# ChenKaiXuSan/Skiing_Analysis_PyTorch

Measured on AMD Instinct MI355X. Metric: 3D-pose frames/sec, 8-view 518px clips, higher is better.
Workload: dtype f16

## Files before the change

include/skimi.h:

```cpp
#ifndef SKIMI_H
#define SKIMI_H

#include <stddef.h>
#include <stdint.h>

#ifdef __cplusplus
extern "C" {
#endif

#define SKIMI_OK 0
#define SKIMI_ERR_ARG (-1)
#define SKIMI_ERR_HIP (-2)
#define SKIMI_ERR_STATE (-3)
#define SKIMI_ERR_WORKSPACE (-4)

#define SKIMI_F32 0
#define SKIMI_BF16 1
#define SKIMI_BF16X3_REC 2
#define SKIMI_FP8MX 3
#define SKIMI_F16 4

#define SKIMI_PREC_BF16 0
#define SKIMI_PREC_BF16X3 1
#define SKIMI_PREC_FP8 2
#define SKIMI_PREC_F16 3

#define SKIMI_ACT_NONE 0
#define SKIMI_ACT_RELU 1
#define SKIMI_ACT_GELU 2
#define SKIMI_ACT_SILU 3
#define SKIMI_ACT_SIGMOID 4

const char* skimi_last_error(void);
int skimi_version(void);
int skimi_sizeof_gemm_desc(void);
int skimi_device_count(void);

int skimi_profile_start(int32_t kind, int64_t min_size);
int skimi_profile_stop(double* total_ms, int64_t* launches, double* flops, double* bytes);

typedef struct skimi_gemm_desc {
    int32_t M, N, K;
    const void* A;
    const void* W;
    int32_t a_dtype, w_dtype;
    int64_t lda, ldw;
    int32_t prec;
    int32_t a_mode;
    int32_t cN, cH, cW, cC, KH, KW, stride, pad, dil, OH, OW;
    const float* bias;
    const float* gamma;
    const void* resid;
    int32_t resid_dtype;
    int64_t ldr;
    int32_t resid_rows_per_batch;
    int64_t resid_batch_stride;
    int64_t resid_row_off;
    int32_t act;
    const void* resid2;
    int64_t ldr2;
    int32_t post_act;
    int32_t out_rows_per_batch;
    int64_t out_batch_stride;
    int64_t out_row_off;
    void* out;
    void* out2;
    int32_t out_dtype;
    int64_t ldo, ldo2;
    int32_t store_mode, ps_s, ps_C;
    void* splitk_scratch;
    uint64_t splitk_scratch_bytes;
    int32_t force_splitk;
    int32_t splitk_scratch_zeroed;
    const void* W_split;
    void* x3_scratch;
    uint64_t x3_scratch_bytes;
    void* out_records;
} skimi_gemm_desc;

int skimi_split_planes(const float* x, int64_t ld, int64_t rows, int32_t C, void* hi, void* lo, void* stream);

int skimi_split_records(const float* x, int64_t ld, int64_t rows, int32_t C, void* records, void* stream);

int skimi_dpt_fold_pack(const float* w_T, const float* b_T, const float* w_rn, int32_t C_in, int32_t C_mid, int32_t C_out,
                        int32_t s, void* w_records, float* beta, void* stream);

int skimi_gemm(const skimi_gemm_desc* d, void* stream);

#define SKIMI_GEMM_PATH_GENERIC 1
#define SKIMI_GEMM_PATH_SPLITK_ORDERED 2
#define SKIMI_GEMM_PATH_SPLITK_ATOMIC 3
#define SKIMI_GEMM_PATH_X3DMA_WIDE 4
#define SKIMI_GEMM_PATH_X3DMA_NARROW 5
#define SKIMI_GEMM_PATH_GEMM256 6
#define SKIMI_GEMM_PATH_CONV_WIN 7
int32_t skimi_gemm_last_path(void);

int skimi_quant_mx(const void* x, int32_t dtype, int64_t ldx, int64_t rows, int32_t K, void* payload, void* scales,
                   void* stream);
int skimi_layernorm_mx(const float* x, int64_t ldx, int64_t rows, int32_t C, const float* gamma, const float* beta,
                       float eps, void* payload, void* scales, void* stream);
int skimi_gemm_fp8(const void* A, const void* A_scales, const void* W, const void* W_scales, int32_t M, int32_t N,
                   int32_t K, const float* bias, int32_t act, const float* gamma, const float* resid, int64_t ldr,
                   void* out, int32_t out_dtype, int64_t ldo, void* out_scales, void* stream);

int skimi_conv3x3_n32_pack(const float* w, void* packed, int32_t C, void* stream);
int skimi_conv3x3_n32(const void* in_hi, const void* in_lo, const void* packed_w, const float* bias, float* out,
                      int32_t F, int32_t H, int32_t W, int32_t C, int32_t relu, void* stream);

int skimi_resample_u8(const uint8_t* in, uint8_t* out, int64_t outer, int32_t n_in, int32_t n_out, int64_t inner,
                      const int32_t* kk, const int32_t* bounds, int32_t ksize, void* stream);
int skimi_u8_hwc_to_f32_chw(const uint8_t* in, int32_t H, int32_t W, float* out, int32_t OH, int32_t OW, int32_t y_off,
                            int32_t x_off, float fill, void* stream);

int skimi_layernorm(const float* x, const float* x2, int64_t ldx, int64_t rows, int32_t C,
                    const float* gamma, const float* beta, float eps,
                    void* out, int32_t out_dtype, int64_t ldo, void* stream);

int skimi_qknorm_rope(void* qkv, int32_t dtype, int64_t tokens, int32_t heads,
                      const float* qn_w, const float* qn_b, const float* kn_w, const float* kn_b,
                      float eps, const int32_t* pos, const float* rope_cos, const float* rope_sin,
                      int32_t rope_npos, void* stream);

int skimi_attention(const void* qkv, void* out, int32_t dtype, int32_t batch, int32_t seq,
                    int32_t heads, int32_t head_dim, void* stream);
int skimi_attention_out(const void* qkv, void* out, int32_t dtype, int32_t out_dtype, int32_t batch, int32_t seq,
                        int32_t heads, int32_t head_dim, void* stream);

int skimi_qknorm_rope_scaled(void* qkv, int32_t dtype, int64_t tokens, int32_t heads,
                             const float* qn_w, const float* qn_b, const float* kn_w, const float* kn_b,
                             float eps, const int32_t* pos, const float* rope_cos, const float* rope_sin,
                             int32_t rope_npos, float q_scale, int32_t* q_scaled, void* stream);
int skimi_attention_ex(const void* qkv, void* out, int32_t dtype, int32_t out_dtype, int32_t batch, int32_t seq,
                       int32_t heads, int32_t head_dim, int32_t q_prescaled, void* x3_scratch,
                       uint64_t x3_scratch_bytes, int32_t* out_records, void* stream);
uint64_t skimi_attention_x3_scratch_bytes(int64_t tokens, int64_t row_elems);

typedef struct skimi_vp3d skimi_vp3d;

skimi_vp3d* skimi_vp3d_create(int32_t joints_in, int32_t in_features, int32_t joints_out,
                              const int32_t* filter_widths, int32_t n_widths,
                              int32_t channels, int32_t causal);
skimi_vp3d* skimi_vp3d_create_ex(int32_t joints_in, int32_t in_features, int32_t joints_out,
                                 const int32_t* filter_widths, int32_t n_widths,
                                 int32_t channels, int32_t causal, int32_t dense);
void skimi_vp3d_destroy(skimi_vp3d*);
int skimi_vp3d_set_weight(skimi_vp3d*, const char* key, const float* host_data, int64_t n);
int skimi_vp3d_finalize(skimi_vp3d*, int32_t prec);
int32_t skimi_vp3d_receptive_field(const skimi_vp3d*);
size_t skimi_vp3d_workspace_bytes(const skimi_vp3d*, int32_t batch, int32_t frames_in);
int skimi_vp3d_forward(skimi_vp3d*, const float* x, float* out, int32_t batch, int32_t frames_in,
                       void* workspace, size_t workspace_bytes, void* stream);

typedef struct skimi_vggt skimi_vggt;

typedef struct skimi_vggt_config {
    int32_t patch_size, embed_dim, depth, num_heads, num_register_tokens;
    int32_t use_dino;
    int32_t dino_depth, dino_heads, dino_img_size;
    int32_t cam_trunk_depth, cam_heads, cam_iters;
// ... 96 lines not shown
```

skiing_analysis_pytorch_amd/_lib.py:

```python
from __future__ import annotations

import ctypes as C
from pathlib import Path

LIB_PATH = Path(__file__).resolve().parent / "lib" / "libskimi.so"

F32, BF16 = 0, 1
F16 = 4
BF16X3_REC = 2
FP8MX = 3
PREC_BF16, PREC_BF16X3, PREC_FP8 = 0, 1, 2
PREC_F16 = 3
ACT_NONE, ACT_RELU, ACT_GELU, ACT_SILU, ACT_SIGMOID = 0, 1, 2, 3, 4
GEMM_PATH_GENERIC, GEMM_PATH_SPLITK_ORDERED, GEMM_PATH_SPLITK_ATOMIC = 1, 2, 3
GEMM_PATH_X3DMA_WIDE, GEMM_PATH_X3DMA_NARROW, GEMM_PATH_GEMM256, GEMM_PATH_CONV_WIN = 4, 5, 6, 7


class SkimiError(RuntimeError):
    pass


class GemmDesc(C.Structure):

    _fields_ = [
        ("M", C.c_int32), ("N", C.c_int32), ("K", C.c_int32),
        ("A", C.c_void_p), ("W", C.c_void_p),
        ("a_dtype", C.c_int32), ("w_dtype", C.c_int32),
        ("lda", C.c_int64), ("ldw", C.c_int64),
        ("prec", C.c_int32),
        ("a_mode", C.c_int32),
        ("cN", C.c_int32), ("cH", C.c_int32), ("cW", C.c_int32), ("cC", C.c_int32),
        ("KH", C.c_int32), ("KW", C.c_int32), ("stride", C.c_int32), ("pad", C.c_int32),
        ("dil", C.c_int32), ("OH", C.c_int32), ("OW", C.c_int32),
        ("bias", C.c_void_p), ("gamma", C.c_void_p), ("resid", C.c_void_p),
        ("resid_dtype", C.c_int32),
        ("ldr", C.c_int64),
        ("resid_rows_per_batch", C.c_int32),
        ("resid_batch_stride", C.c_int64),
        ("resid_row_off", C.c_int64),
        ("act", C.c_int32),
        ("resid2", C.c_void_p), ("ldr2", C.c_int64), ("post_act", C.c_int32),
        ("out_rows_per_batch", C.c_int32), ("out_batch_stride", C.c_int64), ("out_row_off", C.c_int64),
        ("out", C.c_void_p), ("out2", C.c_void_p),
        ("out_dtype", C.c_int32),
        ("ldo", C.c_int64), ("ldo2", C.c_int64),
        ("store_mode", C.c_int32), ("ps_s", C.c_int32), ("ps_C", C.c_int32),
        ("splitk_scratch", C.c_void_p),
        ("splitk_scratch_bytes", C.c_uint64),
        ("force_splitk", C.c_int32), ("splitk_scratch_zeroed", C.c_int32),
        ("W_split", C.c_void_p), ("x3_scratch", C.c_void_p), ("x3_scratch_bytes", C.c_uint64),
        ("out_records", C.c_void_p),
    ]


_vp = C.c_void_p
_SIGNATURES = {
    "skimi_last_error": (C.c_char_p, []),
    "skimi_version": (C.c_int, []),
    "skimi_sizeof_gemm_desc": (C.c_int, []),
    "skimi_device_count": (C.c_int, []),
    "skimi_profile_start": (C.c_int, [C.c_int32, C.c_int64]),
    "skimi_profile_stop": (C.c_int, [C.POINTER(C.c_double), C.POINTER(C.c_int64), C.POINTER(C.c_double),
                                    C.POINTER(C.c_double)]),
    "skimi_gemm": (C.c_int, [C.POINTER(GemmDesc), _vp]),
    "skimi_gemm_last_path": (C.c_int32, []),
    "skimi_dpt_fold_pack": (C.c_int, [_vp, _vp, _vp, C.c_int32, C.c_int32, C.c_int32, C.c_int32, _vp, _vp, _vp]),
    "skimi_quant_mx": (C.c_int, [_vp, C.c_int32, C.c_int64, C.c_int64, C.c_int32, _vp, _vp, _vp]),
    "skimi_layernorm_mx": (C.c_int, [_vp, C.c_int64, C.c_int64, C.c_int32, _vp, _vp, C.c_float, _vp, _vp, _vp]),
    "skimi_gemm_fp8": (C.c_int, [_vp, _vp, _vp, _vp, C.c_int32, C.c_int32, C.c_int32, _vp, C.c_int32, _vp, _vp, C.c_int64,
                                 _vp, C.c_int32, C.c_int64, _vp, _vp]),
    "skimi_split_planes": (C.c_int, [_vp, C.c_int64, C.c_int64, C.c_int32, _vp, _vp, _vp]),
    "skimi_split_records": (C.c_int, [_vp, C.c_int64, C.c_int64, C.c_int32, _vp, _vp]),
    "skimi_resample_u8": (C.c_int, [_vp, _vp, C.c_int64, C.c_int32, C.c_int32, C.c_int64, _vp, _vp, C.c_int32, _vp]),
    "skimi_u8_hwc_to_f32_chw": (C.c_int, [_vp, C.c_int32, C.c_int32, _vp, C.c_int32, C.c_int32, C.c_int32, C.c_int32,
                                          C.c_float, _vp]),
    "skimi_conv3x3_n32_pack": (C.c_int, [_vp, _vp, C.c_int32, _vp]),
    "skimi_conv3x3_n32": (C.c_int, [_vp, _vp, _vp, _vp, _vp, C.c_int32, C.c_int32, C.c_int32, C.c_int32, C.c_int32, _vp]),
    "skimi_layernorm": (C.c_int, [_vp, _vp, C.c_int64, C.c_int64, C.c_int32, _vp, _vp, C.c_float, _vp,
                                  C.c_int32, C.c_int64, _vp]),
    "skimi_qknorm_rope": (C.c_int, [_vp, C.c_int32, C.c_int64, C.c_int32, _vp, _vp, _vp, _vp, C.c_float,
                                    _vp, _vp, _vp, C.c_int32, _vp]),
    "skimi_attention": (C.c_int, [_vp, _vp, C.c_int32, C.c_int32, C.c_int32, C.c_int32, C.c_int32, _vp]),
    "skimi_attention_out": (C.c_int, [_vp, _vp, C.c_int32, C.c_int32, C.c_int32, C.c_int32, C.c_int32, C.c_int32, _vp]),
    "skimi_qknorm_rope_scaled": (C.c_int, [_vp, C.c_int32, C.c_int64, C.c_int32, _vp, _vp, _vp, _vp, C.c_float,
                                           _vp, _vp, _vp, C.c_int32, C.c_float, C.POINTER(C.c_int32), _vp]),
    "skimi_attention_ex": (C.c_int, [_vp, _vp, C.c_int32, C.c_int32, C.c_int32, C.c_int32, C.c_int32, C.c_int32, C.c_int32,
                                     _vp, C.c_uint64, C.POINTER(C.c_int32), _vp]),
    "skimi_attention_x3_scratch_bytes": (C.c_uint64, [C.c_int64, C.c_int64]),
    "skimi_vp3d_create": (_vp, [C.c_int32, C.c_int32, C.c_int32, C.POINTER(C.c_int32), C.c_int32,
                                C.c_int32, C.c_int32]),
    "skimi_vp3d_create_ex": (_vp, [C.c_int32, C.c_int32, C.c_int32, C.POINTER(C.c_int32), C.c_int32,
                                   C.c_int32, C.c_int32, C.c_int32]),
    "skimi_vp3d_destroy": (None, [_vp]),
    "skimi_vp3d_set_weight": (C.c_int, [_vp, C.c_char_p, _vp, C.c_int64]),
    "skimi_vp3d_finalize": (C.c_int, [_vp, C.c_int32]),
    "skimi_vp3d_receptive_field": (C.c_int32, [_vp]),
    "skimi_vp3d_workspace_bytes": (C.c_size_t, [_vp, C.c_int32, C.c_int32]),
    "skimi_vp3d_forward": (C.c_int, [_vp, _vp, _vp, C.c_int32, C.c_int32, _vp, C.c_size_t, _vp]),
    "skimi_pose_to_cameras": (C.c_int, [_vp, C.c_int64, C.c_int32, C.c_int32, _vp, _vp, _vp]),
    "skimi_unproject_depth": (C.c_int, [_vp, _vp, _vp, _vp, C.c_int32, C.c_int32, C.c_int32, _vp]),
    "skimi_triangulate_dlt": (C.c_int, [_vp, _vp, _vp, _vp, _vp, C.c_int64, C.c_int32, C.c_int32, _vp]),
    "skimi_triangulate_triage": (C.c_int, [_vp, _vp, _vp, _vp, _vp, C.c_double, C.c_double, C.c_int64, C.c_int32, C.c_int32,
                                           _vp, _vp, _vp, _vp, _vp, _vp, _vp, _vp]),
    "skimi_triangulate_robust": (C.c_int, [_vp, _vp, _vp, _vp, _vp, C.c_double, C.c_double, C.c_int32, C.c_int32, C.c_int32,
                                           C.c_int64, C.c_int32, C.c_int32, _vp, _vp, _vp, _vp, _vp, _vp, _vp, _vp, _vp]),
    "skimi_person_workspace_bytes": (C.c_size_t, [C.c_int64, C.c_int32, C.c_int32]),
    "skimi_person_origin": (C.c_int, [_vp, _vp, C.c_int64, C.c_int32, C.c_int32, C.c_int32, C.c_int32, _vp, _vp, _vp]),
    "skimi_recenter_cameras": (C.c_int, [_vp, _vp, C.c_int64, C.c_int32, _vp, _vp, _vp, _vp]),
    "skimi_icp_workspace_bytes": (C.c_size_t, [C.c_int64, C.c_int64]),
    "skimi_estimate_normals": (C.c_int, [_vp, C.c_int64, C.c_double, _vp, _vp, _vp, C.c_size_t, _vp]),
    "skimi_icp_correspondences": (C.c_int, [_vp, C.c_int64, _vp, C.c_int64, C.POINTER(C.c_double), C.c_double, _vp, _vp,
                                            C.c_size_t, _vp]),
    "skimi_icp_point_to_plane": (C.c_int, [_vp, C.c_int64, _vp, C.c_int64, C.c_double, C.c_double, C.c_int32, C.c_double,
                                           C.c_double, C.POINTER(C.c_double), C.POINTER(C.c_double), C.POINTER(C.c_double),
                                           C.POINTER(C.c_double), C.POINTER(C.c_int32), _vp, C.c_size_t, _vp]),
    "skimi_ba_workspace_bytes": (C.c_size_t, [C.c_int64, C.c_int32, C.c_int32, C.c_int32]),
    "skimi_bundle_adjust": (C.c_int, [_vp, _vp, _vp, _vp, _vp, _vp, C.c_int64, C.c_int32, C.c_int32, C.POINTER(C.c_int32),
                                      C.c_int32, C.c_int32, C.c_double, C.c_double, C.c_double, C.c_double, C.c_double,
                                      C.c_double, C.c_int32, _vp, _vp, _vp, _vp, _vp, C.c_size_t, _vp]),
    "skimi_resect_workspace_bytes": (C.c_size_t, [C.c_int64, C.c_int32, C.c_int64]),
    "skimi_resect_cameras": (C.c_int, [_vp, _vp, _vp, _vp, _vp, _vp, C.c_int64, C.c_int32, C.c_int64, C.c_int32, C.c_double,
                                       C.c_double, C.c_int32, _vp, _vp, _vp, _vp, _vp, _vp, _vp, _vp, _vp, _vp, _vp, C.c_size_t,
                                       _vp]),
    "skimi_relative_pose": (C.c_int, [_vp, _vp, C.c_int64, C.c_int32, _vp, _vp, _vp]),
    "skimi_vggt_create": (_vp, [_vp]),
    "skimi_vggt_destroy": (None, [_vp]),
    "skimi_vggt_set_weight": (C.c_int, [_vp, C.c_char_p, _vp, C.c_int64, C.c_int32]),
    "skimi_vggt_finalize": (C.c_int, [_vp]),
    "skimi_vggt_set_pos_embed": (C.c_int, [_vp, C.c_int32, C.c_int32, _vp, C.c_int32]),
    "skimi_vggt_rope_positions": (C.c_int, [_vp, C.c_int32, C.c_int32, C.c_int32, _vp]),
    "skimi_vggt_workspace_bytes": (C.c_size_t, [_vp, C.c_int32, C.c_int32, C.c_int32, C.c_int32, C.c_int32]),
    "skimi_vggt_forward": (C.c_int, [_vp, _vp, _vp, C.c_int32, C.c_int32, C.c_int32, C.c_int32, C.c_int32, _vp,
                                     _vp, C.c_size_t, _vp]),
}
# ... 51 lines not shown
```

skiing_analysis_pytorch_amd/csrc/gemm.hip:

```cpp
#include "common.h"
#include "gemm_epilogue.h"
#include <algorithm>
#include <stdlib.h>

namespace skimi {

#define SKIMI_ENV_FLAG(NAME) ([]() { static const bool v = getenv(NAME) && atoi(getenv(NAME)); return v; }())

template <typename T> struct Stage;
template <> struct Stage<float> { float4 a, b; };
template <> struct Stage<unsigned short> { bf16x8 v; };

__device__ __forceinline__ void stage_load(Stage<float>& s, const float* p) {
    s.a = *reinterpret_cast<const float4*>(p);
    s.b = *reinterpret_cast<const float4*>(p + 4);
}
__device__ __forceinline__ void stage_load(Stage<unsigned short>& s, const unsigned short* p) {
    s.v = *reinterpret_cast<const bf16x8*>(p);
}
__device__ __forceinline__ void stage_mask(Stage<float>& s, bool ok) {
    s.a.x = ok ? s.a.x : 0.f; s.a.y = ok ? s.a.y : 0.f; s.a.z = ok ? s.a.z : 0.f; s.a.w = ok ? s.a.w : 0.f;
    s.b.x = ok ? s.b.x : 0.f; s.b.y = ok ? s.b.y : 0.f; s.b.z = ok ? s.b.z : 0.f; s.b.w = ok ? s.b.w : 0.f;
}
__device__ __forceinline__ void stage_mask(Stage<unsigned short>& s, bool ok) {
// ... 317 lines not shown
        if (p.splitk_ordered) {
            for (int sk = 1; sk < p.splitk; ++sk) {
                float* q = p.partial + (long)sk * total + idx;
                v += *q;
                *q = 0.f;
            }
        }
        store_one(p, rm, n, v);
    }
}

template <int BM, int BN, int BK, int NSPLIT, typename TA, typename TW, bool F16 = false>
static int launch_cfg(const GemmArgs& a, hipStream_t st) {
    constexpr int DEPTH = (BM == 64 && BN == 64) ? 4 : 1;
    constexpr int NPL = (NSPLIT == 3) ? 2 : 1;
    constexpr size_t lds = 2ull * NPL * (BM + BN) * BK * 2;
    auto kfn = gemm_kernel<BM, BN, BK, NSPLIT, TA, TW, DEPTH, F16>;
    SKIMI_LDS_OPT_IN(kfn, lds, "gemm");
    dim3 grid(a.ntm * a.ntn, a.splitk);
    hipLaunchKernelGGL(kfn, grid, dim3(256), lds, st, a);
    SKIMI_LAUNCH_CHECK();
    return SKIMI_OK;
}

static thread_local int tl_gemm_path = 0;
void set_gemm_path(int family, int tile, int mfma, int epi, int splitk) {
    tl_gemm_path = family | (tile << 4) | (mfma << 8) | (epi << 12) | (splitk << 16);
}
int gemm_last_path() { return tl_gemm_path; }

int gemm_dispatch(const skimi_gemm_desc* d, hipStream_t st, void* scratch, size_t scratch_bytes,
                  int force_splitk) {
    tl_gemm_path = 0;
    SKIMI_CHECK_ARG(d != nullptr, "skimi_gemm: null descriptor");
    SKIMI_CHECK_ARG(d->M > 0 && d->N > 0 && d->K > 0, "skimi_gemm: empty shape M=%d N=%d K=%d", d->M, d->N, d->K);
    SKIMI_CHECK_ARG(d->K % 8 == 0, "skimi_gemm: K=%d must be a multiple of 8", d->K);
    SKIMI_CHECK_ARG(d->A && d->W && (d->out || d->out_records), "skimi_gemm: null buffer");
    const bool fold = d->a_mode == 3 || d->store_mode == 2;
    if (fold) {
        SKIMI_CHECK_ARG(d->a_mode == 3 && d->store_mode == 2, "skimi_gemm: a_mode 3 and store_mode 2 come together");
        SKIMI_CHECK_ARG(d->cC > 0 && d->cC % 32 == 0 && d->K == 4 * d->cC && (long)d->cN * d->cH * d->cW == d->M &&
                            d->ps_s >= 2 && d->N == d->ps_C && d->N % 32 == 0 && d->lda >= d->cC,
                        "skimi_gemm: bad phase-folded geometry (K = 4 cC, M = cN cH cW, N = ps_C, ps_s >= 2)");
        SKIMI_CHECK_ARG(gemm_x3dma_eligible(d),
                        "skimi_gemm: the phase-folded ConvTranspose + 3x3 conv runs on the 256-column LDS-DMA bf16x3 kernel only "
                        "(W_split, the 9-class bias table, fp32 out / records, ReLU or no activation, ps_C > 128, cW >= 2, a "
                        "chip's worth of tiles)");
    }
    if (d->out_records) {
        SKIMI_CHECK_ARG(d->N % 32 == 0 && (d->store_mode == 0 || fold) && d->out_rows_per_batch == 0 && d->out_row_off == 0 &&
                            d->out2 == nullptr && ((uintptr_t)d->out_records & 127) == 0,
                        "skimi_gemm: out_records needs N %% 32 == 0, plain output rows, no out2, 128-byte alignment");
        SKIMI_CHECK_ARG(d->out || d->out_dtype == SKIMI_F32, "skimi_gemm: records-only output is written from fp32 results");
        SKIMI_CHECK_ARG(d->prec == SKIMI_PREC_BF16X3, "skimi_gemm: out_records is an output form of the fp32-accurate mode");
    }
    SKIMI_CHECK_ARG(d->lda % 4 == 0 && d->ldw % 8 == 0 && d->lda >= 0,
                    "skimi_gemm: lda/ldw must keep 16-B alignment (lda=%ld ldw=%ld)", (long)d->lda, (long)d->ldw);
    SKIMI_CHECK_ARG(!((d->a_dtype == SKIMI_BF16 || d->a_dtype == SKIMI_F16) && d->lda % 8 != 0), "skimi_gemm: 16-bit lda must be a multiple of 8");
    SKIMI_CHECK_ARG(d->prec == SKIMI_PREC_BF16 || d->prec == SKIMI_PREC_BF16X3 || d->prec == SKIMI_PREC_F16, "skimi_gemm: bad prec %d", d->prec);
    {
        const int bad = d->prec == SKIMI_PREC_F16 ? SKIMI_BF16 : SKIMI_F16;
        SKIMI_CHECK_ARG(d->a_dtype != bad && d->w_dtype != bad, "skimi_gemm: prec %d does not take %s operands", d->prec,
                        bad == SKIMI_BF16 ? "bf16" : "fp16");
        SKIMI_CHECK_ARG(d->prec == SKIMI_PREC_F16 || (d->out_dtype != SKIMI_F16), "skimi_gemm: fp16 output belongs to SKIMI_PREC_F16");
        SKIMI_CHECK_ARG(d->out_dtype == SKIMI_F32 || d->out_dtype == SKIMI_BF16 || d->out_dtype == SKIMI_F16, "skimi_gemm: bad out_dtype %d", d->out_dtype);
    }
    const int BK = d->prec == SKIMI_PREC_BF16X3 ? 32 : 64;
    if (d->a_mode != 0 && !fold) {
        SKIMI_CHECK_ARG(d->cC % BK == 0, "skimi_gemm: conv gather needs cC %% %d == 0 (cC=%d)", BK, d->cC);
        SKIMI_CHECK_ARG(d->a_mode != 2 || BK == 32, "skimi_gemm: slice-major conv weights (a_mode 2) need a K-tile of 32 (fp32-accurate mode)");
        SKIMI_CHECK_ARG(d->K == d->KH * d->KW * d->cC, "skimi_gemm: K != KH*KW*cC");
        SKIMI_CHECK_ARG((long)d->cN * d->OH * d->OW == d->M, "skimi_gemm: M != cN*OH*OW");
        SKIMI_CHECK_ARG((d->OH - 1) * d->stride - d->pad + (d->KH - 1) * d->dil < d->cH + d->pad &&
                        (d->OW - 1) * d->stride - d->pad + (d->KW - 1) * d->dil < d->cW + d->pad,
                        "skimi_gemm: conv window exceeds padded input");
        SKIMI_CHECK_ARG(d->lda >= d->cC, "skimi_gemm: conv pixel stride lda < cC");
    }
    if (d->store_mode == 1) {
        SKIMI_CHECK_ARG(d->ps_s > 0 && d->ps_C > 0 && d->N == d->ps_s * d->ps_s * d->ps_C &&
                        (long)d->cN * d->cH * d->cW == d->M, "skimi_gemm: bad pixel-shuffle store geometry");
    }
    if (d->resid) SKIMI_CHECK_ARG(d->ldr >= d->N, "skimi_gemm: ldr < N");
    if (d->resid2) SKIMI_CHECK_ARG(d->ldr2 >= d->N, "skimi_gemm: ldr2 < N");

    GemmArgs a;
    a.M = d->M; a.N = d->N; a.K = d->K;
    a.A = d->A; a.W = d->W; a.lda = d->lda; a.ldw = d->ldw;
    a.a_mode = d->a_mode;
    a.cN = d->cN; a.cH = d->cH; a.cW = d->cW; a.cC = d->cC; a.KH = d->KH; a.KW = d->KW;
    a.stride = d->stride; a.pad = d->pad; a.dil = d->dil; a.OH = d->OH; a.OW = d->OW;
    a.bias = d->bias; a.gamma = d->gamma; a.resid = d->resid; a.ldr = d->ldr; a.resid_dtype = d->resid_dtype;
    a.resid_rpb = d->resid_rows_per_batch; a.resid_bs = d->resid_batch_stride; a.resid_off = d->resid_row_off;
    a.resid2 = d->resid2; a.ldr2 = d->ldr2;
    a.out_rpb = d->out_rows_per_batch; a.out_bs = d->out_batch_stride; a.out_off = d->out_row_off;
    a.post_act = d->post_act;
    a.act = d->act;
    a.out = d->out; a.out2 = d->out2; a.out_dtype = d->out_dtype; a.ldo = d->ldo; a.ldo2 = d->ldo2;
    a.store_mode = d->store_mode; a.ps_s = d->ps_s; a.ps_C = d->ps_C;
    a.out_rec = (unsigned short*)d->out_records;
    a.rec_row = (long)(d->N / 32) * 64;
    a.partial = nullptr;
    a.f16 = d->prec == SKIMI_PREC_F16;
    a.splitk_ordered = 0;
    {
        auto al16 = [](const void* q) { return ((uintptr_t)q & 15) == 0; };
        const bool out_ok = d->out_dtype == SKIMI_F32 ? al16(d->out) : (((uintptr_t)d->out & 7) == 0);
        const bool out2_ok = !d->out2 || (d->out_dtype == SKIMI_F32 ? (((uintptr_t)d->out2 & 7) == 0) : al16(d->out2));
        a.vec4 = (d->N % 4 == 0) && (d->ldo % 4 == 0) && (!d->out2 || d->ldo2 % 4 == 0) && out_ok && out2_ok &&
                 (!d->bias || al16(d->bias)) && (!d->gamma || al16(d->gamma)) &&
                 (!d->resid || ((((uintptr_t)d->resid) & 7) == 0 && (d->resid_dtype != SKIMI_F32 || al16(d->resid)) && d->ldr % 4 == 0)) &&
                 (!d->resid2 || ((((uintptr_t)d->resid2) & 7) == 0 && (d->resid_dtype != SKIMI_F32 || al16(d->resid2)) && d->ldr2 % 4 == 0)) && (d->store_mode == 0 || d->ps_C % 4 == 0);
    }

    if (force_splitk <= 0 && gemm_x3dma_eligible(d)) {
        a.partial = nullptr;
        a.k_per_split = d->K;
        return gemm_x3dma_launch(a, d, st);
    }
    if (d->out_records &&
        hipMemsetAsync((char*)d->out_records + (size_t)d->M * (d->N / 32) * 128, 0, 256, st) != hipSuccess) {
        set_error("hipMemsetAsync(out_records zero page) failed");
        return SKIMI_ERR_HIP;
    }
    SKIMI_CHECK_ARG(d->a_dtype != SKIMI_BF16X3_REC,
                    "skimi_gemm: A given as bf16x3 records, but the launch does not qualify for the LDS-DMA kernel "
                    "(M=%d N=%d: needs W_split, M >= 4096, N >= 96, most of a chip's worth of 256-row tiles (>= 160), a zero page behind A)", d->M, d->N);

    if (force_splitk <= 0 && gemm256_eligible(d)) {
        a.partial = nullptr;
        a.k_per_split = d->K;
        const bool prof256 = prof_armed(PROF_GEMM, (long)d->M);
        if (prof256) prof_before(st);
        int rc256 = gemm256_launch(a, st);
        if (prof256)
            prof_after(st, 2.0 * d->M * (double)d->N * d->K,
                       2.0 * d->M * (double)d->K + 2.0 * d->N * (double)d->K +
                           (d->out_dtype == SKIMI_F32 ? 4.0 : 2.0) * d->M * (double)d->N);
        return rc256;
    }

    if (force_splitk <= 0 && conv_win_eligible(d)) {
        set_gemm_path(SKIMI_GEMM_PATH_CONV_WIN, 0, 0, 0, 1);
        const bool profw = prof_armed(PROF_GEMM, (long)d->M);
        if (profw) prof_before(st);
        const int rcw = conv_win_launch(a, st);
        if (profw)
            prof_after(st, 2.0 * d->M * (double)d->N * d->K,
                       2.0 * d->M * (double)d->cC + 2.0 * d->N * (double)d->K + (d->out_dtype == SKIMI_F32 ? 4.0 : 2.0) * d->M * (double)d->N);
        return rcw;
    }

    const long t128 = cdiv(d->M, 128) * cdiv(d->N, 128);
    const bool small = t128 < 128;
    const int BM = small ? 64 : 128;
    const int BN = (BM == 128 && d->N <= 64) ? 64 : BM;
    a.ntm = (int)cdiv(d->M, BM);
    a.ntn = (int)cdiv(d->N, BN);
    const long tiles = (long)a.ntm * a.ntn;
    int splitk = 1;
    const int nkt = (int)cdiv(d->K, BK);
    bool ordered = !SKIMI_ENV_FLAG("SKIMI_SPLITK_ATOMIC");
    const size_t plane = (size_t)d->M * d->N * sizeof(float);
    if (force_splitk > 0) {
        splitk = force_splitk;
        if (ordered && plane * (size_t)splitk > scratch_bytes) ordered = false;
    } else if (tiles < 192 && nkt >= 8 && scratch != nullptr && plane <= scratch_bytes) {
        splitk = (int)std::min<long>(cdiv(512, tiles), nkt / 4);
        if (ordered) splitk = (int)std::min<size_t>((size_t)splitk, scratch_bytes / plane);
        if (splitk < 1) splitk = 1;
    }
    int kper = (int)cdiv(nkt, splitk) * BK;
    splitk = (int)cdiv(d->K, kper);
    a.splitk = splitk;
    a.k_per_split = kper;
    a.splitk_ordered = ordered && splitk > 1;
    if (splitk > 1) {
        size_t need = plane * (a.splitk_ordered ? (size_t)splitk : 1);
        if (scratch == nullptr || need > scratch_bytes) {
            set_error("skimi_gemm: split-K scratch too small (%zu needed, %zu given)", need, scratch_bytes);
            return SKIMI_ERR_WORKSPACE;
        }
        a.partial = (float*)scratch;
        if (!d->splitk_scratch_zeroed) SKIMI_HIP(hipMemsetAsync(scratch, 0, need, st));
    }
    set_gemm_path(splitk == 1 ? SKIMI_GEMM_PATH_GENERIC : a.splitk_ordered ? SKIMI_GEMM_PATH_SPLITK_ORDERED : SKIMI_GEMM_PATH_SPLITK_ATOMIC,
                  BM == 64 ? 1 : BN == 64 ? 2 : 3, 0, 0, splitk);
// ... 76 lines not shown
```

skiing_analysis_pytorch_amd/csrc/gemm256.hip:

```cpp
#include <stdlib.h>

#include "common.h"
#include "gemm_epilogue.h"

namespace skimi {

typedef __attribute__((address_space(3))) void lds_void;
typedef __attribute__((address_space(1))) const void gbl_void;

__device__ __forceinline__ void tile_coords256(const GemmArgs& p, int& tm, int& tn) {
    const int nblk = p.ntm * p.ntn;
    const int bid = blockIdx.x;
    const int xcd = bid & 7;
    const int q = nblk >> 3, r = nblk & 7;
    const int id = (xcd < r ? xcd * (q + 1) : r * (q + 1) + (xcd - r) * q) + (bid >> 3);
    constexpr int GM = 8;
    const int per_group = GM * p.ntn;
    const int group = id / per_group, within = id - group * per_group;
    const int rows = min(GM, p.ntm - group * GM);
    tn = within / rows;
    tm = group * GM + within - tn * rows;
}

template <bool H16>
__device__ __forceinline__ bf16x4 pack4_16(float y0, float y1, float y2, float y3) {
    bf16x4 hb;
    if constexpr (H16) {
        hb[0] = (short)f2h(y0); hb[1] = (short)f2h(y1); hb[2] = (short)f2h(y2); hb[3] = (short)f2h(y3);
    } else {
        hb[0] = (short)f2bf(y0); hb[1] = (short)f2bf(y1); hb[2] = (short)f2bf(y2); hb[3] = (short)f2bf(y3);
    }
    return hb;
}

template <int MT>
__device__ __forceinline__ void acc_to_slab(float* stg, const f32x16 (&acc)[MT][2], int i, int lane) {
    const int l31 = lane & 31, lh = lane >> 5;
#pragma unroll
    for (int j = 0; j < 2; ++j)
#pragma unroll
        for (int r = 0; r < 16; ++r) stg[((r & 3) + 8 * (r >> 2) + 4 * lh) * 64 + j * 32 + l31] = acc[i][j][r];
}
template <int MT>
__device__ __forceinline__ void acc_to_slab(float* stg, const f32x4 (&acc)[2 * MT][4], int i, int lane) {
    const int l15 = lane & 15, lq = lane >> 4;
#pragma unroll
    for (int b = 0; b < 2; ++b)
#pragma unroll
        for (int c = 0; c < 4; ++c)
#pragma unroll
            for (int r = 0; r < 4; ++r) stg[(16 * b + 4 * lq + r) * 64 + 16 * c + l15] = acc[2 * i + b][c][r];
}

template <int MT, int EPI, int PF = 2, bool H16 = false, typename ACC>
__device__ __forceinline__ void epilogue256(const GemmArgs& p, ACC& acc, char* smem, int wave, int lane,
                                            int wr, int wc, int m0, int n0) {
    float* stg = reinterpret_cast<float*>(smem) + wave * (32 * 64);
    const int n = n0 + wc * 64 + 4 * (lane & 15);
    if (p.dbg & 8) {
        if (acc[0][0][0] == 123.456f) ((float*)p.out)[0] = acc[MT - 1][1][sizeof(acc[0][0]) / 4 - 1];
        return;
    }
    const bool interior = (m0 + 64 * MT <= p.M) && (n0 + 256 <= p.N) && !(p.dbg & 4);
    float4 bs = make_float4(0, 0, 0, 0), gm = make_float4(1, 1, 1, 1);
    if (EPI != 0 && n < p.N) {
        if (p.bias) bs = *reinterpret_cast<const float4*>(p.bias + n);
        if (EPI == 2) gm = *reinterpret_cast<const float4*>(p.gamma + n);
    }
#define SKIMI_ACC_TO_SLAB(i)                                                                                   \
    do {                                                                                                        \
        acc_to_slab<MT>(stg, acc, i, lane);                                                                     \
        __builtin_amdgcn_fence(__ATOMIC_RELEASE, "wavefront");                                                  \
        __builtin_amdgcn_s_waitcnt(0xC07F);                                                     \
    } while (0)

    if (EPI == 2 && interior) {
        const int mrow0 = m0 + wr * (32 * MT) + (lane >> 4);
        float4 r[PF][8];
#pragma unroll
        for (int i = 0; i < PF && i < MT; ++i)
#pragma unroll
            for (int it = 0; it < 8; ++it)
                r[i][it] = *reinterpret_cast<const float4*>((const float*)p.resid + (long)(mrow0 + i * 32 + it * 4) * p.ldr + n);
#pragma unroll
        for (int i = 0; i < MT; ++i) {
            SKIMI_ACC_TO_SLAB(i);
            const int mrow = mrow0 + i * 32;
            float4 v[8];
#pragma unroll
            for (int it = 0; it < 8; ++it)
                v[it] = *reinterpret_cast<const float4*>(&stg[(it * 4 + (lane >> 4)) * 64 + 4 * (lane & 15)]);
#pragma unroll
            for (int it = 0; it < 8; ++it) {
                const float4 rr = r[i % PF][it];
                f32x4 ov = {rr.x + gm.x * (v[it].x + bs.x), rr.y + gm.y * (v[it].y + bs.y),
                            rr.z + gm.z * (v[it].z + bs.z), rr.w + gm.w * (v[it].w + bs.w)};
                *reinterpret_cast<f32x4*>((float*)p.out + (long)(mrow + it * 4) * p.ldo + n) = ov;
            }
            if (i + PF < MT) {
#pragma unroll
                for (int it = 0; it < 8; ++it)
                    r[i % PF][it] =
                        *reinterpret_cast<const float4*>((const float*)p.resid + (long)(mrow + PF * 32 + it * 4) * p.ldr + n);
            }
            __builtin_amdgcn_s_waitcnt(0xC07F);
        }
        return;
    }
    if (EPI != 0 && interior) {
        const bool mx = EPI == 3 && p.out_dtype == SKIMI_FP8MX;
#pragma unroll
        for (int i = 0; i < MT; ++i) {
            SKIMI_ACC_TO_SLAB(i);
            const int mrow = m0 + wr * (32 * MT) + i * 32 + (lane >> 4);
            float4 v[8];
#pragma unroll
            for (int it = 0; it < 8; ++it)
                v[it] = *reinterpret_cast<const float4*>(&stg[(it * 4 + (lane >> 4)) * 64 + 4 * (lane & 15)]);
            unsigned sb_mine = 0;
#pragma unroll
            for (int it = 0; it < 8; ++it) {
                float y0 = v[it].x + bs.x, y1 = v[it].y + bs.y, y2 = v[it].z + bs.z, y3 = v[it].w + bs.w;
                if (EPI == 3) {
                    const f32x2_t g0 = gelu_erf2(f32x2_t{y0, y1}), g1 = gelu_erf2(f32x2_t{y2, y3});
                    y0 = g0.x; y1 = g0.y; y2 = g1.x; y3 = g1.y;
                }
                if (mx) {
                    const unsigned sb = mx_scale_byte(max8(fmaxf(fmaxf(fabsf(y0), fabsf(y1)), fmaxf(fabsf(y2), fabsf(y3)))));
                    const long row = mrow + it * 4;
                    *reinterpret_cast<int*>((unsigned char*)p.out + row * p.ldo + n) = mx_pack4(y0, y1, y2, y3, mx_inv_scale(sb));
                    sb_mine = (lane & 7) == it ? sb : sb_mine;
                    if (it == 7) p.out_scales[(long)(mrow + (lane & 7) * 4) * (p.N >> 5) + (n >> 5)] = (unsigned char)sb_mine;
                    continue;
                }
                *reinterpret_cast<bf16x4*>((unsigned short*)p.out + (long)(mrow + it * 4) * p.ldo + n) = pack4_16<H16>(y0, y1, y2, y3);
            }
            __builtin_amdgcn_s_waitcnt(0xC07F);
        }
        return;
    }
#pragma unroll
    for (int i = 0; i < MT; ++i) {
        SKIMI_ACC_TO_SLAB(i);
// ... 380 lines not shown
#pragma unroll
    for (int h = 0; h < 2; ++h)
#pragma unroll
        for (int i = 0; i < 8; ++i)
#pragma unroll
            for (int c = 0; c < 4; ++c) {
                acc[h][i][c] = f32x4{0.f, 0.f, 0.f, 0.f};
                asm volatile("" : "+a"(acc[h][i][c]));
            }
    asm volatile("s_nop 1");
    auto mfma = [&](f32x4& c, const bf16x8& a, const bf16x8& b) {
        if constexpr (F16) asm volatile("v_mfma_f32_16x16x32_f16 %0, %1, %2, %0" : "+a"(c) : "v"(a), "v"(b));
        else asm volatile("v_mfma_f32_16x16x32_bf16 %0, %1, %2, %0" : "+a"(c) : "v"(a), "v"(b));
    };
    auto kstep = [&](bf16x8 (&fa)[8], bf16x8 (&fb)[8], auto&& extra) {
#pragma unroll
        for (int j = 0; j < 8; ++j)
#pragma unroll
            for (int i = 0; i < 8; ++i) {
                mfma(acc[j >> 2][i][j & 3], fa[i], fb[j]);
                extra(8 * j + i);
                __builtin_amdgcn_sched_barrier(0);
            }
    };

#pragma unroll
    for (int q = 0; q < 4; ++q) issue(q, 0, q);
    if (nkt > 1) {
#pragma unroll
        for (int q = 0; q < 4; ++q) issue(q, 1, 4 + q);
        SKIMI_VMCNT(16);
    } else {
        SKIMI_VMCNT(0);
    }
    SKIMI_BAR();
    int sb = 0;
#pragma unroll
    for (int n = 0; n < 16; ++n) read_one(sb, 0, n, fa0, fb0);
#define SKIMI_W4_HEAD()                       \
    do {                                      \
        __builtin_amdgcn_s_waitcnt(0xC07F);   \
        __builtin_amdgcn_sched_barrier(0);    \
    } while (0)
#define SKIMI_W4_KTILE(N1, N2)                                                                       \
    do {                                                                                             \
        int s8 = sb + 8, s9 = sb + 9, s1 = sb + 1, nsb = sb + 4;                                     \
        s8 = s8 >= NSLOT ? s8 - NSLOT : s8;                                                          \
        s9 = s9 >= NSLOT ? s9 - NSLOT : s9;                                                          \
        s1 = s1 >= NSLOT ? s1 - NSLOT : s1;                                                          \
        nsb = nsb >= NSLOT ? nsb - NSLOT : nsb;                                                      \
                                          \
        SKIMI_W4_HEAD();                                                                             \
        kstep(fa0, fb0, [&](int g) {                                                                 \
            if (g < 16) read_one(sb, 1, g, fa1, fb1);                                                \
            else if (N2 && g < 32 && (g & 1)) {                                              \
                const int d = (g - 16) >> 1;                                                         \
                issue_one(d >> 2, d & 3, kt + 2, (d >> 2) ? s9 : s8);                                \
            }                                                                                        \
        });                                                                                          \
                         \
        SKIMI_W4_HEAD();                                                                             \
        if (N1) {                                                                                    \
            if (N2) SKIMI_VMCNT(8); else SKIMI_VMCNT(0);                                             \
            SKIMI_BAR();                                                                             \
        }                                                                                            \
        kstep(fa1, fb1, [&](int g) {                                                                 \
            if (N1 && g < 16) read_one(nsb, 0, g, fa0, fb0);                                         \
            else if (N2 && g < 32 && (g & 1)) {                                              \
                const int d = (g - 16) >> 1;                                                         \
                issue_one(2 + (d >> 2), d & 3, kt + 2, (d >> 2) ? s1 : sb);                          \
            }                                                                                        \
        });                                                                                          \
        sb = nsb;                                                                                    \
    } while (0)
    int kt = 0;
    for (; kt + 2 < nkt; ++kt) SKIMI_W4_KTILE(true, true);
    if (kt + 1 < nkt) {
        SKIMI_W4_KTILE(true, false);
        ++kt;
    }
    SKIMI_W4_KTILE(false, false);
#undef SKIMI_W4_KTILE
#undef SKIMI_W4_HEAD
    asm volatile("s_nop 7\n\ts_nop 4");
#pragma unroll
    for (int h = 0; h < 2; ++h)
#pragma unroll
        for (int i = 0; i < 8; ++i)
#pragma unroll
            for (int c = 0; c < 4; ++c) asm volatile("" : "+a"(acc[h][i][c]));
    __builtin_amdgcn_s_waitcnt(0xC07F);
    SKIMI_BAR();

    epilogue256<4, EPI, 4, F16 && EPI == 3>(p, acc[0], smem, wave, lane, wr, 2 * wc, m0, n0);
    epilogue256<4, EPI, 4, F16 && EPI == 3>(p, acc[1], smem, wave, lane, wr, 2 * wc + 1, m0, n0);
    } else {
    const int t = lh ^ ((l31 >> 1) & 7);
    const int lane_off = l31 * RB;
    bf16x8 fa0[4], fb0[4], fa1[4], fb1[4];
    auto read = [&](int sb, int s, bf16x8 (&fa)[4], bf16x8 (&fb)[4]) {
        int sa = sb + wr, sw = sb + 2 + wc;
        sa = sa >= NSLOT ? sa - NSLOT : sa;
        sw = sw >= NSLOT ? sw - NSLOT : sw;
        const char* pa = smem + sa * PIECE + lane_off + (((2 * s) ^ t) << 4);
        const char* pw = smem + sw * PIECE + lane_off + (((2 * s) ^ t) << 4);
#pragma unroll
        for (int i = 0; i < 4; ++i) fa[i] = *reinterpret_cast<const bf16x8*>(pa + i * 32 * RB);
#pragma unroll
        for (int i = 0; i < 4; ++i) fb[i] = *reinterpret_cast<const bf16x8*>(pw + i * 32 * RB);
    };

    f32x16 acc[2][4][2];
#pragma unroll
    for (int h = 0; h < 2; ++h)
#pragma unroll
        for (int i = 0; i < 4; ++i)
#pragma unroll
            for (int j = 0; j < 2; ++j)
#pragma unroll
                for (int r = 0; r < 16; ++r) acc[h][i][j][r] = 0.f;
#define SKIMI_W4_MFMA(FA, FB)                                                                                   \
    _Pragma("unroll") for (int j = 0; j < 4; ++j) _Pragma("unroll") for (int i = 0; i < 4; ++i)                 \
        acc[j >> 1][i][j & 1] = mfma_32x32x16<F16>(FA[i], FB[j], acc[j >> 1][i][j & 1])

#pragma unroll
    for (int q = 0; q < 4; ++q) issue(q, 0, q);
    if (nkt > 1) {
#pragma unroll
        for (int q = 0; q < 4; ++q) issue(q, 1, 4 + q);
        SKIMI_VMCNT(16);
    } else {
        SKIMI_VMCNT(0);
    }
    SKIMI_BAR();
    int sb = 0;
    read(sb, 0, fa0, fb0);
#define SKIMI_W4_HEAD()                       \
    do {                                      \
        __builtin_amdgcn_s_waitcnt(0xC07F);   \
        __builtin_amdgcn_sched_barrier(0);    \
    } while (0)
#define SKIMI_W4_TAIL(NDMA)                                                        \
    do {                                                                           \
        _Pragma("unroll") for (int g = 0; g < 4; ++g) {                            \
            __builtin_amdgcn_sched_group_barrier(0x008, 1, 0);                     \
            __builtin_amdgcn_sched_group_barrier(0x100, 2, 0);                     \
        }                                                                          \
        _Pragma("unroll") for (int g = 0; g < NDMA; ++g) {                         \
            __builtin_amdgcn_sched_group_barrier(0x008, 1, 0);                     \
            __builtin_amdgcn_sched_group_barrier(0x010, 1, 0);                     \
        }                                                                          \
        __builtin_amdgcn_sched_group_barrier(0x008, 12 - NDMA, 0);                 \
        __builtin_amdgcn_sched_barrier(0);                                         \
    } while (0)
#define SKIMI_W4_KTILE(N1, N2)                                                      \
    do {                                                                            \
        int s8 = sb + 8, s9 = sb + 9, s1 = sb + 1, nsb = sb + 4;                    \
        s8 = s8 >= NSLOT ? s8 - NSLOT : s8;                                         \
        s9 = s9 >= NSLOT ? s9 - NSLOT : s9;                                         \
        s1 = s1 >= NSLOT ? s1 - NSLOT : s1;                                         \
        nsb = nsb >= NSLOT ? nsb - NSLOT : nsb;                                     \
                                                                      \
        SKIMI_W4_HEAD();                                                            \
        read(sb, 1, fa1, fb1);                                                      \
        SKIMI_W4_MFMA(fa0, fb0);                                                    \
        SKIMI_W4_TAIL(0);                                                           \
                                                                      \
        SKIMI_W4_HEAD();                                                            \
        read(sb, 2, fa0, fb0);                                                      \
        if (N2) issue(0, kt + 2, s8);                                               \
        SKIMI_W4_MFMA(fa1, fb1);                                                    \
        SKIMI_W4_TAIL((N2 ? 4 : 0));                                                \
                                                                      \
        SKIMI_W4_HEAD();                                                            \
        read(sb, 3, fa1, fb1);                                                      \
        if (N2) issue(1, kt + 2, s9);                                               \
        SKIMI_W4_MFMA(fa0, fb0);                                                    \
        SKIMI_W4_TAIL((N2 ? 4 : 0));                                                \
                                                                      \
        SKIMI_W4_HEAD();                                                            \
        if (N1) {                                                                   \
            if (N2) SKIMI_VMCNT(8); else SKIMI_VMCNT(0);                            \
            SKIMI_BAR();                                                            \
            read(nsb, 0, fa0, fb0);                                                 \
            if (N2) {                                                               \
                issue(2, kt + 2, sb);                                               \
                issue(3, kt + 2, s1);                                               \
            }                                                                       \
        }                                                                           \
        SKIMI_W4_MFMA(fa1, fb1);                                                    \
        if (N1) SKIMI_W4_TAIL((N2 ? 8 : 0)); else __builtin_amdgcn_sched_barrier(0); \
        sb = nsb;                                                                   \
    } while (0)
    int kt = 0;
    for (; kt + 2 < nkt; ++kt) SKIMI_W4_KTILE(true, true);
    if (kt + 1 < nkt) {
        SKIMI_W4_KTILE(true, false);
        ++kt;
    }
    SKIMI_W4_KTILE(false, false);
#undef SKIMI_W4_KTILE
#undef SKIMI_W4_HEAD
#undef SKIMI_W4_TAIL
#undef SKIMI_W4_MFMA
    __builtin_amdgcn_s_waitcnt(0xC07F);
    SKIMI_BAR();

    epilogue256<4, EPI, 4, F16 && EPI == 3>(p, acc[0], smem, wave, lane, wr, 2 * wc, m0, n0);
    epilogue256<4, EPI, 4, F16 && EPI == 3>(p, acc[1], smem, wave, lane, wr, 2 * wc + 1, m0, n0);
    }
}


typedef __attribute__((ext_vector_type(8))) int i32x8_t;
typedef __attribute__((ext_vector_type(4))) int i32x4_t;

template <int EPI>
__global__ __launch_bounds__(256, 1) void gemm256w4_fp8_kernel(const GemmArgs p) {
    constexpr int RB = 128, BK = 128, PIECE = 128 * RB, NSLOT = 10;
    extern __shared__ __attribute__((aligned(16))) char smem[];

    const int tid = threadIdx.x, lane = tid & 63;
    const int wave = __builtin_amdgcn_readfirstlane(tid >> 6);
    const int wr = wave >> 1, wc = wave & 1;
    const int l31 = lane & 31, lh = lane >> 5;

    int tm, tn;
    tile_coords256(p, tm, tn);
    const int m0 = tm * 256, n0 = tn * 256;
    const int nkt = p.K / BK;
    const unsigned char* src[4][4];
#pragma unroll
    for (int q = 0; q < 4; ++q)
#pragma unroll
        for (int j = 0; j < 4; ++j) {
            const int row = (4 * wave + j) * 8 + (lane >> 3);
            const int c = (lane & 7) ^ ((row >> 1) & 7);
            src[q][j] = q < 2 ? (const unsigned char*)p.A + (long)min(m0 + 128 * q + row, p.M - 1) * p.lda + c * 16
                              : (const unsigned char*)p.W + (long)min(n0 + 128 * (q - 2) + row, p.N - 1) * p.ldw + c * 16;
        }
    auto issue = [&](int q, int kt, int slot) {
        char* base = smem + slot * PIECE + (4 * wave) * 8 * RB;
#pragma unroll
        for (int j = 0; j < 4; ++j)
            __builtin_amdgcn_global_load_lds((gbl_void*)(src[q][j] + (long)kt * BK), (lds_void*)(base + j * 8 * RB), 16, 0, 0);
    };
    const unsigned* asc[4];
    const unsigned* wsc[4];
#pragma unroll
    for (int i = 0; i < 4; ++i) {
        asc[i] = reinterpret_cast<const unsigned*>(p.a_scales + (long)min(m0 + 128 * wr + 32 * i + l31, p.M - 1) * p.lsa);
        wsc[i] = reinterpret_cast<const unsigned*>(p.w_scales + (long)min(n0 + 128 * wc + 32 * i + l31, p.N - 1) * p.lsw);
    }
    unsigned sa[4], sw[4], san[4], swn[4];
    auto load_scales = [&](int kt) {
#pragma unroll
        for (int i = 0; i < 4; ++i) {
            san[i] = asc[i][kt];
            swn[i] = wsc[i][kt];
        }
    };
    auto take_scales = [&]() {
#pragma unroll
        for (int i = 0; i < 4; ++i) {
            sa[i] = san[i] >> (8 * lh);
            sw[i] = swn[i] >> (8 * lh);
        }
    };

    const int t = lh ^ ((l31 >> 1) & 7);
    const int lane_off = l31 * RB;
    i32x4_t fa0[2][4], fb0[2][4], fa1[2][4], fb1[2][4];
    auto readp = [&](int sb, int ks, i32x4_t (&fa)[2][4], i32x4_t (&fb)[2][4]) {
        int sA = sb + wr, sW = sb + 2 + wc;
        sA = sA >= NSLOT ? sA - NSLOT : sA;
        sW = sW >= NSLOT ? sW - NSLOT : sW;
#pragma unroll
        for (int h = 0; h < 2; ++h) {
            const int s = 2 * ks + h;
            const char* pa = smem + sA * PIECE + lane_off + (((2 * s) ^ t) << 4);
            const char* pw = smem + sW * PIECE + lane_off + (((2 * s) ^ t) << 4);
#pragma unroll
            for (int i = 0; i < 4; ++i) fa[h][i] = *reinterpret_cast<const i32x4_t*>(pa + i * 32 * RB);
#pragma unroll
            for (int i = 0; i < 4; ++i) fb[h][i] = *reinterpret_cast<const i32x4_t*>(pw + i * 32 * RB);
        }
    };

    f32x16 acc[2][4][2];
#pragma unroll
// ... 53 lines not shown
        readp(sb, 1, fa1, fb1);                                                     \
        if (N2) {                                                                   \
            issue(0, kt + 2, s8);                                                   \
            issue(1, kt + 2, s9);                                                   \
        }                                                                           \
        SKIMI_F8_MFMA(fa0, fb0, 0);                                                 \
        SKIMI_F8_TAIL((N2 ? 8 : 0));                                                \
                                                  \
        SKIMI_F8_HEAD();                                                            \
        if (N1) {                                                                   \
            if (N2) SKIMI_VMCNT(8); else SKIMI_VMCNT(0);                            \
            SKIMI_BAR();                                                            \
            readp(nsb, 0, fa0, fb0);                                                \
            load_scales(kt + 1);                                                    \
            if (N2) {                                                               \
                issue(2, kt + 2, sb);                                               \
                issue(3, kt + 2, s1);                                               \
            }                                                                       \
        }                                                                           \
        SKIMI_F8_MFMA(fa1, fb1, 2);                                                 \
        if (N1) SKIMI_F8_TAIL((N2 ? 16 : 8)); else __builtin_amdgcn_sched_barrier(0); \
        if (N1) {                                                                   \
            SKIMI_VMCNT(PW);            \
            take_scales();                                                          \
        }                                                                           \
        sb = nsb;                                                                   \
    } while (0)
    int kt = 0;
    for (; kt + 2 < nkt; ++kt) SKIMI_F8_KTILE(true, true, 8);
    if (kt + 1 < nkt) {
        SKIMI_F8_KTILE(true, false, 0);
        ++kt;
    }
    SKIMI_F8_KTILE(false, false, 0);
#undef SKIMI_F8_KTILE
#undef SKIMI_F8_HEAD
#undef SKIMI_F8_TAIL
#undef SKIMI_F8_MFMA
#undef SKIMI_F8_CAT
    __builtin_amdgcn_s_waitcnt(0xC07F);
    SKIMI_BAR();

    epilogue256<4, EPI, 4>(p, acc[0], smem, wave, lane, wr, 2 * wc, m0, n0);
    epilogue256<4, EPI, 4>(p, acc[1], smem, wave, lane, wr, 2 * wc + 1, m0, n0);
}

static int env_int(const char* name, int dflt, int& cache, bool& have) {
    static const bool dynamic = getenv("SKIMI_ENV_DYNAMIC") && atoi(getenv("SKIMI_ENV_DYNAMIC"));
    if (!have || dynamic) {
        const char* v = getenv(name);
        cache = v ? atoi(v) : dflt;
        have = true;
    }
    return cache;
}
#define SKIMI_ENV_INT(NAME, DFLT) ([]() { static int c; static bool h = false; return env_int(NAME, DFLT, c, h); }())

static int epi_kind(const GemmArgs& a) {
    const bool plain = a.vec4 && a.store_mode == 0 && a.out_rpb == 0 && a.out_off == 0 && a.out2 == nullptr &&
                       a.resid2 == nullptr && a.post_act == SKIMI_ACT_NONE && a.N % 4 == 0;
    if (!plain) return 0;
    if (a.gamma == nullptr && a.resid == nullptr && (a.out_dtype == SKIMI_BF16 || a.out_dtype == SKIMI_F16)) {
        if (a.act == SKIMI_ACT_NONE && a.out_dtype == SKIMI_BF16) return 1;
        if (a.act == SKIMI_ACT_GELU && a.out_dtype == (a.f16 ? SKIMI_F16 : SKIMI_BF16)) return 3;
        return 0;
    }
    if (a.out_dtype == SKIMI_FP8MX && a.out_scales != nullptr && a.gamma == nullptr && a.resid == nullptr && a.bias != nullptr &&
        a.act == SKIMI_ACT_GELU && a.N % 128 == 0)
        return 3;
    if (a.out_dtype == SKIMI_F32 && a.gamma != nullptr && a.resid != nullptr && a.resid_dtype == SKIMI_F32 &&
        a.resid_rpb == 0 && a.resid_off == 0 && a.act == SKIMI_ACT_NONE)
        return 2;
    return 0;
}

bool gemm256_eligible(const skimi_gemm_desc* d) {
    const bool bf = d->prec == SKIMI_PREC_BF16 && d->a_dtype == SKIMI_BF16 && d->w_dtype == SKIMI_BF16;
    const bool hf = d->prec == SKIMI_PREC_F16 && d->a_dtype == SKIMI_F16 && d->w_dtype == SKIMI_F16;
    return (bf || hf) && d->a_mode == 0 &&
           d->store_mode == 0 && d->K % 64 == 0 && d->lda % 8 == 0 && d->ldw % 8 == 0 && d->M >= 2048 &&
           d->N >= 512 && (((uintptr_t)d->A | (uintptr_t)d->W) & 15) == 0;
}

template <int MT, int EPI, bool F16 = false>
static int launch256(GemmArgs& a, hipStream_t st) {
    constexpr size_t lds = 2ull * (64 * MT + 256) * 128;
    SKIMI_LDS_OPT_IN((gemm256_kernel<MT, EPI, F16>), lds, "gemm256");
    a.ntm = (int)cdiv(a.M, 64 * MT);
    a.ntn = (int)cdiv(a.N, 256);
    a.splitk = 1;
    hipLaunchKernelGGL((gemm256_kernel<MT, EPI, F16>), dim3(a.ntm * a.ntn), dim3(512), lds, st, a);
    SKIMI_LAUNCH_CHECK();
    return SKIMI_OK;
}

template <int EPI, int DEEP, bool F16, bool M16>
static int launch256pp_(GemmArgs& a, hipStream_t st) {
    constexpr size_t lds = 2ull * (256 + 256) * 128;
    SKIMI_LDS_OPT_IN((gemm256pp_kernel<EPI, DEEP, F16, M16>), lds, "gemm256pp");
    a.ntm = (int)cdiv(a.M, 256);
    a.ntn = (int)cdiv(a.N, 256);
    a.splitk = 1;
    hipLaunchKernelGGL((gemm256pp_kernel<EPI, DEEP, F16, M16>), dim3(a.ntm * a.ntn), dim3(512), lds, st, a);
    SKIMI_LAUNCH_CHECK();
    return SKIMI_OK;
}

template <int EPI, bool F16, bool M16>
static int launch256pp(GemmArgs& a, hipStream_t st) {
    if constexpr (F16) return launch256pp_<EPI, 1, true, M16>(a, st);
    const int deep = SKIMI_ENV_INT("SKIMI_GEMM256_DEEP", 1);
    return deep ? launch256pp_<EPI, 1, false, M16>(a, st) : launch256pp_<EPI, 0, false, M16>(a, st);
}

template <int EPI, bool F16, bool M16>
static int launch256w4(GemmArgs& a, hipStream_t st) {
    constexpr size_t lds = 10ull * 128 * 128;
    SKIMI_LDS_OPT_IN((gemm256w4_kernel<EPI, F16, M16>), lds, "gemm256w4");
    a.ntm = (int)cdiv(a.M, 256);
    a.ntn = (int)cdiv(a.N, 256);
    a.splitk = 1;
    hipLaunchKernelGGL((gemm256w4_kernel<EPI, F16, M16>), dim3(a.ntm * a.ntn), dim3(256), lds, st, a);
    SKIMI_LAUNCH_CHECK();
    return SKIMI_OK;
}

template <bool F16, bool M16>
static int gemm256_pick_loop(GemmArgs& a, hipStream_t st, int epi, bool w4) {
    if (w4) {
        if (epi == 1) return launch256w4<1, F16, M16>(a, st);
        if (epi == 2) return launch256w4<2, F16, M16>(a, st);
        if (epi == 3) return launch256w4<3, F16, M16>(a, st);
        return launch256w4<0, F16, M16>(a, st);
    }
    if (epi == 1) return launch256pp<1, F16, M16>(a, st);
    if (epi == 2) return launch256pp<2, F16, M16>(a, st);
    if (epi == 3) return launch256pp<3, F16, M16>(a, st);
    return launch256pp<0, F16, M16>(a, st);
}

template <bool F16>
static int gemm256_pick(GemmArgs& a, hipStream_t st, int epi, bool mt3, bool w4, int use_pp, bool m16) {
    if (mt3) {
        if (epi == 1) return launch256<3, 1, F16>(a, st);
        if (epi == 2) return launch256<3, 2, F16>(a, st);
        if (epi == 3) return launch256<3, 3, F16>(a, st);
        return launch256<3, 0, F16>(a, st);
    }
    if (w4 || use_pp || F16) return m16 ? gemm256_pick_loop<F16, true>(a, st, epi, w4) : gemm256_pick_loop<F16, false>(a, st, epi, w4);
    if constexpr (!F16) {
        if (epi == 1) return launch256<4, 1>(a, st);
        if (epi == 2) return launch256<4, 2>(a, st);
        if (epi == 3) return launch256<4, 3>(a, st);
        return launch256<4, 0>(a, st);
    }
    return SKIMI_ERR_ARG;
}

int gemm256_launch(GemmArgs& a, hipStream_t st) {
#ifdef SKIMI_ABLATIONS
    a.dbg = SKIMI_ENV_INT("SKIMI_GEMM256_ABL", 0);
#else
    a.dbg = 0;
#endif
    auto cost = [&](int bm) {
        const long tiles = cdiv(a.M, bm) * cdiv(a.N, 256);
        return (double)cdiv(tiles, 256) * bm;
    };
    const int epi = epi_kind(a);
    const bool m16 = SKIMI_ENV_INT("SKIMI_GEMM256_MFMA", 16) != 32;
    const int use_pp = SKIMI_ENV_INT("SKIMI_GEMM256_PP", 1);
    const int use_mt3 = SKIMI_ENV_INT("SKIMI_GEMM256_MT3", -1);
    const int use_w4 = SKIMI_ENV_INT("SKIMI_GEMM256_W4", -1);
    const bool mt3 = use_mt3 == 1 || (use_mt3 < 0 && cost(192) < 0.8 * cost(256));
    const bool w4 = use_w4 >= 0 ? use_w4 != 0 : (epi == 1 || (epi == 2 && a.K > 1024));
    const int loop = mt3 ? 2 : w4 ? 4 : (use_pp || a.f16) ? 3 : 1;
    set_gemm_path(SKIMI_GEMM_PATH_GEMM256, loop, (loop >= 3 && m16) ? 1 : 2, epi, 1);
    return a.f16 ? gemm256_pick<true>(a, st, epi, mt3, w4, use_pp, m16) : gemm256_pick<false>(a, st, epi, mt3, w4, use_pp, m16);
}

template <int EPI>
static int launch256w4_fp8(GemmArgs& a, hipStream_t st) {
    constexpr size_t lds = 10ull * 128 * 128;
    SKIMI_LDS_OPT_IN(gemm256w4_fp8_kernel<EPI>, lds, "gemm256w4_fp8");
    a.ntm = (int)cdiv(a.M, 256);
    a.ntn = (int)cdiv(a.N, 256);
    a.splitk = 1;
    hipLaunchKernelGGL((gemm256w4_fp8_kernel<EPI>), dim3(a.ntm * a.ntn), dim3(256), lds, st, a);
    SKIMI_LAUNCH_CHECK();
    return SKIMI_OK;
}

int gemm256_fp8_launch(GemmArgs& a, hipStream_t st) {
    a.dbg = 0;
    const int epi = epi_kind(a);
    if (epi == 1) return launch256w4_fp8<1>(a, st);
    if (epi == 2) return launch256w4_fp8<2>(a, st);
    if (epi == 3) return launch256w4_fp8<3>(a, st);
    set_error("gemm256_fp8: epilogue not supported");
    return SKIMI_ERR_ARG;
}

}
```

skiing_analysis_pytorch_amd/csrc/gemm_epilogue.h:

```cpp
#pragma once
#include "common.h"

namespace skimi {

struct GemmArgs {
    int M, N, K;
    const void* A;
    const void* W;
    long lda, ldw;
    int a_mode;
    int cN, cH, cW, cC, KH, KW, stride, pad, dil, OH, OW;
    const float* bias;
    const float* gamma;
    const void* resid;
    int resid_dtype;
    long ldr;
    int resid_rpb;
    long resid_bs;
    long resid_off;
    const void* resid2;
    long ldr2;
    int out_rpb;
    long out_bs;
    long out_off;
    int act;
    int post_act;
    void* out;
    void* out2;
    int out_dtype;
    long ldo, ldo2;
    int store_mode, ps_s, ps_C;
    int splitk;
    int k_per_split;
    float* partial;
    int splitk_ordered;
    int ntm, ntn;
    int vec4;
    int f16;
    int dbg;
    unsigned short* out_rec;
    long rec_row;
    const unsigned char* a_scales;
    const unsigned char* w_scales;
    long lsa, lsw;
    unsigned char* out_scales;
};

__device__ __forceinline__ void store_rec4(const GemmArgs& p, long m, int n, float v0, float v1, float v2, float v3) {
    const float f[4] = {v0, v1, v2, v3};
    bf16x4 h, l;
#pragma unroll
    for (int k = 0; k < 4; ++k) {
        const unsigned short hb = f2bf(f[k]);
        h[k] = (short)hb;
        l[k] = (short)f2bf(f[k] - bf2f(hb));
    }
    unsigned short* q = p.out_rec + m * p.rec_row + (n >> 5) * 64 + (n & 31);
    *reinterpret_cast<bf16x4*>(q) = h;
    *reinterpret_cast<bf16x4*>(q + 32) = l;
}

__device__ __forceinline__ float gelu_erf(float v) {
    const float z = fabsf(v) * 0.70710678118654752440f;
    const float t = __builtin_amdgcn_rcpf(__builtin_fmaf(0.3275911f, z, 1.f));
    float q = __builtin_fmaf(t, 1.061405429f, -1.453152027f);
    q = __builtin_fmaf(t, q, 1.421413741f);
    q = __builtin_fmaf(t, q, -0.284496736f);
    q = __builtin_fmaf(t, q, 0.254829592f);
    q = q * t * __builtin_amdgcn_exp2f(-1.4426950408889634f * z * z) * 0.5f;
    return v >= 0.f ? __builtin_fmaf(-v, q, v) : v * q;
}
typedef float f32x2_t __attribute__((ext_vector_type(2)));
__device__ __forceinline__ f32x2_t gelu_erf2(f32x2_t v) {
    const f32x2_t a = {fabsf(v.x), fabsf(v.y)};
    const f32x2_t d = a * 0.23164190165f + 1.f;
    const f32x2_t t = {__builtin_amdgcn_rcpf(d.x), __builtin_amdgcn_rcpf(d.y)};
    const f32x2_t w = a * 0.84932180028f;
    const f32x2_t ww = w * w;
    const f32x2_t e = {__builtin_amdgcn_exp2f(-ww.x), __builtin_amdgcn_exp2f(-ww.y)};
    f32x2_t q = t * 0.5307027145f + (-0.7265760135f);
    q = t * q + 0.7107068705f;
    q = t * q + (-0.142248368f);
    q = t * q + 0.127414796f;
    q = q * t * e;
    const f32x2_t relu = {fmaxf(v.x, 0.f), fmaxf(v.y, 0.f)};
    return relu - a * q;
}
__device__ __forceinline__ float sigmoid_hw(float v) {
    return __builtin_amdgcn_rcpf(1.f + __builtin_amdgcn_exp2f(-1.4426950408889634f * v));
}
__device__ __forceinline__ float apply_act(float v, int act) {
    switch (act) {
        case SKIMI_ACT_RELU: return fmaxf(v, 0.f);
        case SKIMI_ACT_GELU: return gelu_erf(v);
        case SKIMI_ACT_SILU: return v * sigmoid_hw(v);
        case SKIMI_ACT_SIGMOID: return sigmoid_hw(v);
        default: return v;
    }
}

__device__ __forceinline__ float load_res(const void* r, int dt, long i) {
    return dt == SKIMI_F32 ? ((const float*)r)[i] : x16tof(((const unsigned short*)r)[i], dt == SKIMI_F16);
}
__device__ __forceinline__ float4 load_res4(const void* r, int dt, long i) {
    if (dt == SKIMI_F32) return *reinterpret_cast<const float4*>((const float*)r + i);
    const bf16x4 v = *reinterpret_cast<const bf16x4*>((const unsigned short*)r + i);
    const bool h = dt == SKIMI_F16;
    return make_float4(x16tof((unsigned short)v[0], h), x16tof((unsigned short)v[1], h), x16tof((unsigned short)v[2], h),
                       x16tof((unsigned short)v[3], h));
}

struct RowMap {
    long out_off;
    long out2_off;
    long res_off;
    long res2_off;
    long row;
};

__device__ __forceinline__ RowMap row_map(const GemmArgs& p, int m) {
    RowMap r;
    r.row = m;
    if (p.store_mode == 0) {
        long mo = m;
        if (p.out_rpb > 0) {
            int b = m / p.out_rpb;
            mo = (long)b * p.out_bs + (m - b * p.out_rpb);
        }
// ... 36 lines not shown
        int ab = n / p.ps_C;
        int co = n - ab * p.ps_C;
        int a = ab / p.ps_s;
        int b = ab - a * p.ps_s;
        long OWs = (long)p.cW * p.ps_s;
        long pix = rm.out_off + (long)a * OWs + b;
        o = pix * p.ldo + co;
        o2 = pix * p.ldo2 + co;
    }
    if (p.out_rec) {
        const unsigned short hb = f2bf(v);
        unsigned short* q = p.out_rec + rm.row * p.rec_row + (n >> 5) * 64 + (n & 31);
        q[0] = hb;
        q[32] = f2bf(v - bf2f(hb));
    }
    if (!p.out) return;
    if (p.out_dtype == SKIMI_F32) {
        ((float*)p.out)[o] = v;
        if (p.out2) ((unsigned short*)p.out2)[o2] = f2bf(v);
    } else {
        ((unsigned short*)p.out)[o] = f2x16(v, p.out_dtype == SKIMI_F16);
        if (p.out2) ((float*)p.out2)[o2] = v;
    }
}

__device__ __forceinline__ void store_four(const GemmArgs& p, const RowMap& rm, int n, float4 acc) {
    float v[4] = {acc.x, acc.y, acc.z, acc.w};
    if (p.bias) {
        const float4 b = *reinterpret_cast<const float4*>(p.bias + n);
        v[0] += b.x; v[1] += b.y; v[2] += b.z; v[3] += b.w;
    }
#pragma unroll
    for (int k = 0; k < 4; ++k) v[k] = apply_act(v[k], p.act);
    if (p.gamma) {
        const float4 g = *reinterpret_cast<const float4*>(p.gamma + n);
        v[0] *= g.x; v[1] *= g.y; v[2] *= g.z; v[3] *= g.w;
    }
    if (p.resid) {
        const float4 r = load_res4(p.resid, p.resid_dtype, rm.res_off + n);
        v[0] += r.x; v[1] += r.y; v[2] += r.z; v[3] += r.w;
    }
    if (p.resid2) {
        const float4 r = load_res4(p.resid2, p.resid_dtype, rm.res2_off + n);
        v[0] += r.x; v[1] += r.y; v[2] += r.z; v[3] += r.w;
    }
    if (p.post_act != SKIMI_ACT_NONE) {
#pragma unroll
        for (int k = 0; k < 4; ++k) v[k] = apply_act(v[k], p.post_act);
    }
    long o, o2;
    if (p.store_mode == 0) {
        o = rm.out_off + n;
        o2 = rm.out2_off + n;
    } else {
        int ab = n / p.ps_C;
        int co = n - ab * p.ps_C;
        int a = ab / p.ps_s;
        int b = ab - a * p.ps_s;
        long OWs = (long)p.cW * p.ps_s;
        long pix = rm.out_off + (long)a * OWs + b;
        o = pix * p.ldo + co;
        o2 = pix * p.ldo2 + co;
    }
    if (p.out_rec) store_rec4(p, rm.row, n, v[0], v[1], v[2], v[3]);
    if (!p.out) return;
    bf16x4 hb;
    const bool h16 = p.out_dtype == SKIMI_F16;
#pragma unroll
    for (int k = 0; k < 4; ++k) hb[k] = (short)f2x16(v[k], h16);
    const float4 fv = make_float4(v[0], v[1], v[2], v[3]);
    if (p.out_dtype == SKIMI_F32) {
        *reinterpret_cast<float4*>((float*)p.out + o) = fv;
        if (p.out2) *reinterpret_cast<bf16x4*>((unsigned short*)p.out2 + o2) = hb;
    } else {
        *reinterpret_cast<bf16x4*>((unsigned short*)p.out + o) = hb;
        if (p.out2) *reinterpret_cast<float4*>((float*)p.out2 + o2) = fv;
    }
}

void set_gemm_path(int family, int tile, int mfma, int epi, int splitk);
int gemm_last_path();

bool gemm256_eligible(const skimi_gemm_desc* d);
bool gemm_x3dma_eligible(const skimi_gemm_desc* d);
int gemm_x3dma_launch(GemmArgs& a, const skimi_gemm_desc* d, hipStream_t st);
size_t gemm_x3dma_scratch_bytes(const skimi_gemm_desc* d);
int split_planes_launch(const float* x, long ld, long rows, int C, void* hi, void* lo, hipStream_t st);
int split_records_launch(const float* x, long ld, long rows, int C, void* rec, hipStream_t st, void* zpage = nullptr);
int gemm256_launch(GemmArgs& a, hipStream_t st);
bool conv_win_eligible(const skimi_gemm_desc* d);
int conv_win_launch(GemmArgs& a, hipStream_t st);
int gemm256_fp8_launch(GemmArgs& a, hipStream_t st);

}
```

skiing_analysis_pytorch_amd/csrc/rowops.hip:

```cpp
#include <algorithm>

#include "common.h"
#include "kernels.h"

namespace skimi {

template <int MAXV>
__global__ __launch_bounds__(256) void layernorm_kernel(const float* __restrict__ x,
                                                        const float* __restrict__ x2, long ldx, long rows,
                                                        int C, const float* __restrict__ gamma,
                                                        const float* __restrict__ beta, float eps, void* out,
                                                        int out_dtype, long ldo, long grp_rows,
                                                        long grp_stride, long grp_off) {
    const int lane = threadIdx.x & 63;
    const long orow = (long)blockIdx.x * 4 + (threadIdx.x >> 6);
    if (orow >= rows) return;
    const long row = grp_rows > 0 ? (orow / grp_rows) * grp_stride + grp_off + orow % grp_rows : orow;
    const int half = C >> 1;
    float v[MAXV];
    float s = 0.f;
#pragma unroll
    for (int i = 0; i < MAXV; ++i) {
        const int c = lane + 64 * i;
        float t = 0.f;
        if (c < C) {
            if (x2 == nullptr) t = x[row * ldx + c];
            else t = (c < half) ? x[row * ldx + c] : x2[row * ldx + (c - half)];
        }
        v[i] = t;
        s += t;
    }
    const float mean = wave_sum(s) / (float)C;
    float q = 0.f;
#pragma unroll
    for (int i = 0; i < MAXV; ++i) {
        const int c = lane + 64 * i;
        const float d = (c < C) ? (v[i] - mean) : 0.f;
        q += d * d;
    }
    const float rstd = rsqrtf(wave_sum(q) / (float)C + eps);
#pragma unroll
    for (int i = 0; i < MAXV; ++i) {
        const int c = lane + 64 * i;
        if (c < C) {
            float y = (v[i] - mean) * rstd;
            if (gamma) y *= gamma[c];
            if (beta) y += beta[c];
            if (out_dtype == SKIMI_F32) ((float*)out)[orow * ldo + c] = y;
            else ((unsigned short*)out)[orow * ldo + c] = f2x16(y, out_dtype == SKIMI_F16);
        }
    }
}

template <int NV>
__global__ __launch_bounds__(256) void layernorm_vec_kernel(const float* __restrict__ x, const float* __restrict__ x2,
                                                            long ldx, long rows, const float* __restrict__ gamma,
                                                            const float* __restrict__ beta, float eps, void* out,
                                                            int out_dtype, long ldo, long grp_rows, long grp_stride,
                                                            long grp_off, unsigned char* __restrict__ out_scales = nullptr) {
    constexpr int C = NV * 256;
    const int lane = threadIdx.x & 63;
    const long orow = (long)blockIdx.x * 4 + (threadIdx.x >> 6);
    if (orow >= rows) return;
    const long row = grp_rows > 0 ? (orow / grp_rows) * grp_stride + grp_off + orow % grp_rows : orow;
    float4 v[NV];
    float s = 0.f;
#pragma unroll
    for (int i = 0; i < NV; ++i) {
        const int c = 256 * i + 4 * lane;
        const float* src = (x2 != nullptr && c >= C / 2) ? x2 + row * ldx + (c - C / 2) : x + row * ldx + c;
        v[i] = *reinterpret_cast<const float4*>(src);
        s += (v[i].x + v[i].y) + (v[i].z + v[i].w);
    }
    const float mean = wave_sum(s) * (1.0f / (float)C);
    float q = 0.f;
#pragma unroll
    for (int i = 0; i < NV; ++i) {
        const float a = v[i].x - mean, b = v[i].y - mean, c2 = v[i].z - mean, d = v[i].w - mean;
        q += (a * a + b * b) + (c2 * c2 + d * d);
    }
    const float rstd = rsqrtf(wave_sum(q) * (1.0f / (float)C) + eps);
#pragma unroll
    for (int i = 0; i < NV; ++i) {
        const int c = 256 * i + 4 * lane;
        float y[4] = {(v[i].x - mean) * rstd, (v[i].y - mean) * rstd, (v[i].z - mean) * rstd, (v[i].w - mean) * rstd};
        if (gamma) {
// ... 134 lines not shown
        pp = min(max(pp, 0), npos - 1);
        const float c = rcos[pp * 16 + (d & 15)];
        const float s = rsin[pp * 16 + (d & 15)];
        const float other = __shfl_xor(t, 16, 64);
        const float rot = (d < 16) ? -other : other;
        t = t * c + rot * s;
    }
    if (sizeof(T) == 4) ((float*)p)[lane] = t;
    else ((unsigned short*)p)[lane] = f2bf(t);
}

template <typename T>
__global__ __launch_bounds__(256) void qknorm_rope_vec_kernel(T* __restrict__ qkv, long tokens, int heads,
                                                              const float* __restrict__ qn_w,
                                                              const float* __restrict__ qn_b,
                                                              const float* __restrict__ kn_w,
                                                              const float* __restrict__ kn_b, float eps,
                                                              const int* __restrict__ pos,
                                                              const float* __restrict__ rcos,
                                                              const float* __restrict__ rsin, int npos) {
    const long gid = (long)blockIdx.x * 256 + threadIdx.x;
    const long vec = gid >> 3;
    const int sub = (int)(gid & 7);
    const long total = tokens * 2 * heads;
    const bool live = vec < total;
    const long vv = live ? vec : total - 1;
    const long tok = vv / (2 * heads);
    const int rem = (int)(vv - tok * 2 * heads);
    const int which = rem / heads;
    const int h = rem - which * heads;
    T* p = qkv + ((tok * 3 + which) * heads + h) * 64 + 8 * sub;
    float t[8];
    if (sizeof(T) == 4) {
        const float4 a = *reinterpret_cast<const float4*>(p), b = *reinterpret_cast<const float4*>((const float*)p + 4);
        t[0] = a.x; t[1] = a.y; t[2] = a.z; t[3] = a.w; t[4] = b.x; t[5] = b.y; t[6] = b.z; t[7] = b.w;
    } else {
        const bf16x8 a = *reinterpret_cast<const bf16x8*>(p);
#pragma unroll
        for (int j = 0; j < 8; ++j) t[j] = bf2f((unsigned short)a[j]);
    }
    const float* w = which ? kn_w : qn_w;
    const float* b = which ? kn_b : qn_b;
    if (w != nullptr) {
        float s = 0.f;
#pragma unroll
        for (int j = 0; j < 8; ++j) s += t[j];
        s += __shfl_xor(s, 1, 64); s += __shfl_xor(s, 2, 64); s += __shfl_xor(s, 4, 64);
        const float mean = s * (1.f / 64.f);
        float q = 0.f;
#pragma unroll
        for (int j = 0; j < 8; ++j) { t[j] -= mean; q += t[j] * t[j]; }
        q += __shfl_xor(q, 1, 64); q += __shfl_xor(q, 2, 64); q += __shfl_xor(q, 4, 64);
        const float rstd = rsqrtf(q * (1.f / 64.f) + eps);
#pragma unroll
        for (int j = 0; j < 8; ++j) t[j] = t[j] * rstd * w[8 * sub + j] + (b ? b[8 * sub + j] : 0.f);
    }
    if (pos != nullptr) {
        const int sect = sub >> 2;
        const int d0 = (8 * sub) & 31;
        int pp = pos[tok * 2 + sect];
        pp = min(max(pp, 0), npos - 1);
        const float* ct = rcos + pp * 16 + (d0 & 15);
        const float* st = rsin + pp * 16 + (d0 & 15);
        const bool lower = d0 < 16;
#pragma unroll
        for (int j = 0; j < 8; ++j) {
            const float other = __shfl_xor(t[j], 2, 64);
            const float rot = lower ? -other : other;
            t[j] = t[j] * ct[j] + rot * st[j];
        }
    }
    if (!live) return;
    if (sizeof(T) == 4) {
        *reinterpret_cast<float4*>(p) = make_float4(t[0], t[1], t[2], t[3]);
        *reinterpret_cast<float4*>((float*)p + 4) = make_float4(t[4], t[5], t[6], t[7]);
    } else {
        bf16x8 o;
#pragma unroll
        for (int j = 0; j < 8; ++j) o[j] = (short)f2bf(t[j]);
        *reinterpret_cast<bf16x8*>(p) = o;
    }
}

__device__ __forceinline__ float dpp_xor1(float v) {
    return __int_as_float(__builtin_amdgcn_update_dpp(0, __float_as_int(v), 0xB1, 0xF, 0xF, true));
}
__device__ __forceinline__ float dpp_xor2(float v) {
    return __int_as_float(__builtin_amdgcn_update_dpp(0, __float_as_int(v), 0x4E, 0xF, 0xF, true));
}
__device__ __forceinline__ float dpp_mirror8(float v) {
    return __int_as_float(__builtin_amdgcn_update_dpp(0, __float_as_int(v), 0x141, 0xF, 0xF, true));
}
__device__ __forceinline__ float sum8(float s) {
    s += dpp_xor1(s);
    s += dpp_xor2(s);
    s += dpp_mirror8(s);
    return s;
}

__global__ __launch_bounds__(256) void qknorm_rope_bf16_kernel(unsigned short* __restrict__ qkv, long tokens, int heads,
                                                               const float* __restrict__ qn_w,
                                                               const float* __restrict__ qn_b,
                                                               const float* __restrict__ kn_w,
                                                               const float* __restrict__ kn_b, float eps,
                                                               const int* __restrict__ pos,
                                                               const float* __restrict__ rcos,
                                                               const float* __restrict__ rsin, int npos, float q_scale) {
    extern __shared__ __attribute__((aligned(16))) float tab[];
    for (int i = threadIdx.x; i < npos * 16; i += 256) {
        tab[i] = rcos[i];
        tab[npos * 16 + i] = rsin[i];
    }
    __syncthreads();
    const int sub = threadIdx.x & 7;
    float w[2][8], b[2][8];
#pragma unroll
    for (int j = 0; j < 8; ++j) {
        w[0][j] = qn_w[8 * sub + j]; b[0][j] = qn_b ? qn_b[8 * sub + j] : 0.f;
        w[1][j] = kn_w[8 * sub + j]; b[1][j] = kn_b ? kn_b[8 * sub + j] : 0.f;
    }
    const int sect = sub >> 2;
    const int d0 = (8 * sub) & 15;
    const bool lower = ((8 * sub) & 31) < 16;
    const long total = tokens * heads;
    const long step = (long)gridDim.x * 32;
    const long trips = (total + step - 1) / step;
    long idx = (long)blockIdx.x * 32 + (threadIdx.x >> 3);
    for (long it = 0; it < trips; ++it, idx += step) {
        const bool live = idx < total;
        const long ii = live ? idx : total - 1;
        const long tok = ii / heads;
        const int h = (int)(ii - tok * heads);
        unsigned short* pq = qkv + ((tok * 3) * heads + h) * 64 + 8 * sub;
        unsigned short* pk = pq + (long)heads * 64;
        const bf16x8 raw[2] = {*reinterpret_cast<const bf16x8*>(pq), *reinterpret_cast<const bf16x8*>(pk)};
        int pp = pos[tok * 2 + sect];
        pp = min(max(pp, 0), npos - 1);
        const float4 c0 = *reinterpret_cast<const float4*>(&tab[pp * 16 + d0]);
        const float4 c1 = *reinterpret_cast<const float4*>(&tab[pp * 16 + d0 + 4]);
        const float4 s0 = *reinterpret_cast<const float4*>(&tab[npos * 16 + pp * 16 + d0]);
        const float4 s1 = *reinterpret_cast<const float4*>(&tab[npos * 16 + pp * 16 + d0 + 4]);
        const float ct[8] = {c0.x, c0.y, c0.z, c0.w, c1.x, c1.y, c1.z, c1.w};
        const float st[8] = {s0.x, s0.y, s0.z, s0.w, s1.x, s1.y, s1.z, s1.w};
        bf16x8 outv[2];
#pragma unroll
        for (int z = 0; z < 2; ++z) {
            float t[8];
#pragma unroll
            for (int j = 0; j < 8; ++j) t[j] = bf2f((unsigned short)raw[z][j]);
            float s = 0.f;
#pragma unroll
            for (int j = 0; j < 8; ++j) s += t[j];
            const float mean = sum8(s) * (1.f / 64.f);
            float q = 0.f;
#pragma unroll
            for (int j = 0; j < 8; ++j) { t[j] -= mean; q += t[j] * t[j]; }
            const float rstd = rsqrtf(sum8(q) * (1.f / 64.f) + eps);
#pragma unroll
            for (int j = 0; j < 8; ++j) t[j] = t[j] * rstd * w[z][j] + b[z][j];
#pragma unroll
            for (int j = 0; j < 8; ++j) {
                const float other = dpp_xor2(t[j]);
                const float rot = lower ? -other : other;
                const float r = t[j] * ct[j] + rot * st[j];
                outv[z][j] = (short)f2bf(z == 0 ? r * q_scale : r);
            }
        }
        if (live) {
            *reinterpret_cast<bf16x8*>(pq) = outv[0];
            *reinterpret_cast<bf16x8*>(pk) = outv[1];
        }
    }
}

int qknorm_rope_launch(void* qkv, int dtype, int64_t tokens, int heads, const float* qn_w, const float* qn_b,
                       const float* kn_w, const float* kn_b, float eps, const int32_t* pos,
                       const float* rope_cos, const float* rope_sin, int rope_npos, hipStream_t st, float q_scale,
                       int* q_scaled) {
    SKIMI_CHECK_ARG(qkv && tokens > 0 && heads > 0, "skimi_qknorm_rope: bad arguments");
    if (q_scaled) *q_scaled = 0;
    SKIMI_CHECK_ARG(pos == nullptr || (rope_cos && rope_sin && rope_npos > 0), "skimi_qknorm_rope: pos without tables");
    if (((uintptr_t)qkv & 15) == 0 && dtype == SKIMI_BF16 && qn_w && kn_w && pos && rope_npos * 128 <= 48 * 1024) {
        const long total = tokens * heads;
        const unsigned blocks = (unsigned)std::min<long>(cdiv(total, 32), 256 * 8);
        hipLaunchKernelGGL(qknorm_rope_bf16_kernel, dim3(blocks), dim3(256), (size_t)rope_npos * 128, st,
                           (unsigned short*)qkv, (long)tokens, heads, qn_w, qn_b, kn_w, kn_b, eps, pos, rope_cos, rope_sin,
                           rope_npos, q_scaled ? q_scale : 1.f);
        if (q_scaled) *q_scaled = 1;
        SKIMI_LAUNCH_CHECK();
        return SKIMI_OK;
    }
    if (((uintptr_t)qkv & 15) == 0) {
        const long threads = tokens * 2 * heads * 8;
        dim3 g((unsigned)cdiv(threads, 256)), blk(256);
        if (dtype == SKIMI_F32)
            hipLaunchKernelGGL(qknorm_rope_vec_kernel<float>, g, blk, 0, st, (float*)qkv, (long)tokens, heads, qn_w, qn_b,
                               kn_w, kn_b, eps, pos, rope_cos, rope_sin, rope_npos);
        else
            hipLaunchKernelGGL(qknorm_rope_vec_kernel<unsigned short>, g, blk, 0, st, (unsigned short*)qkv, (long)tokens,
                               heads, qn_w, qn_b, kn_w, kn_b, eps, pos, rope_cos, rope_sin, rope_npos);
        SKIMI_LAUNCH_CHECK();
        return SKIMI_OK;
    }
    const long total = tokens * 2 * heads;
    dim3 grid((unsigned)cdiv(total, 4)), block(256);
    if (dtype == SKIMI_F32)
        hipLaunchKernelGGL(qknorm_rope_kernel<float>, grid, block, 0, st, (float*)qkv, (long)tokens, heads, qn_w,
                           qn_b, kn_w, kn_b, eps, pos, rope_cos, rope_sin, rope_npos);
    else
        hipLaunchKernelGGL(qknorm_rope_kernel<unsigned short>, grid, block, 0, st, (unsigned short*)qkv,
                           (long)tokens, heads, qn_w, qn_b, kn_w, kn_b, eps, pos, rope_cos, rope_sin, rope_npos);
    SKIMI_LAUNCH_CHECK();
    return SKIMI_OK;
}

__global__ __launch_bounds__(256) void vp3d_im2col_kernel(const float* __restrict__ x, float* __restrict__ a0,
                                                          int B, int L, int Cin, int k, int Kpad) {
    const int Lout = L - k + 1;
    const long total = (long)B * Lout * Kpad;
    for (long i = (long)blockIdx.x * 256 + threadIdx.x; i < total; i += (long)gridDim.x * 256) {
        const int c = (int)(i % Kpad);
        const long r = i / Kpad;
        const int b = (int)(r / Lout);
        const int t = (int)(r - (long)b * Lout);
        a0[i] = (c < k * Cin) ? x[((long)b * L + t) * Cin + c] : 0.f;
    }
}

int vp3d_im2col_launch(const float* x, float* a0, int B, int L, int Cin, int k, int Kpad, hipStream_t st) {
    const long total = (long)B * (L - k + 1) * Kpad;
    int blocks = (int)std::min<long>(cdiv(total, 256), 1024);
    hipLaunchKernelGGL(vp3d_im2col_kernel, dim3(blocks), dim3(256), 0, st, x, a0, B, L, Cin, k, Kpad);
    SKIMI_LAUNCH_CHECK();
    return SKIMI_OK;
}

}
```

skiing_analysis_pytorch_amd/csrc/vggt.hip:

```cpp
#include <math.h>
#include <string.h>

#include <map>
#include <memory>
#include <string>
#include <tuple>
#include <atomic>
#include <mutex>
#include <vector>

#include <stdlib.h>

#include "common.h"
#include "gemm_epilogue.h"
#include "kernels.h"
#include "track_kernels.h"
#include "vggt_kernels.h"

using namespace skimi;

namespace {

struct Lin {
    void* w = nullptr;
// ... 1 lines not shown
    float* b = nullptr;
    int N = 0, K = 0;
    int prec = SKIMI_PREC_BF16X3;
    void* w_split = nullptr;
    void* wq = nullptr;
    void* wq_scales = nullptr;
};
struct LNw { float* g = nullptr; float* b = nullptr; };
struct BlockW {
    LNw n1, n2;
    Lin qkv, proj, fc1, fc2;
    float *ls1 = nullptr, *ls2 = nullptr;
    float *qn_w = nullptr, *qn_b = nullptr, *kn_w = nullptr, *kn_b = nullptr;
};
struct ConvW { Lin lin; int k = 1, stride = 1, pad = 0, cin = 0; int kmode = 1; };
struct FusionW { Lin out_conv; ConvW r1c1, r1c2, r2c1, r2c2; bool has_r1 = false; };
struct DptW {
    LNw norm;
    Lin proj[4];
    Lin rs0, rs1;
    Lin fold[2];
    ConvW rs3;
    ConvW rn[4];
    FusionW ref[4];
    ConvW oc1, oc2a;
    float *oc2b_w = nullptr, *oc2b_b = nullptr;
    unsigned short* oc2a_direct = nullptr;
    int n_out = 0, features = 0, oc[4] = {0, 0, 0, 0};
    bool feature_only = false, pos_embed = true;
    bool out_f32 = false;
    const LNw* out_ln = nullptr;
    int down_ratio = 1;
};
struct CamW {
    std::vector<BlockW> trunk;
    LNw token_norm, trunk_norm;
    float* empty16 = nullptr;
    Lin embed_pose, poseLN, fc1, fc2;
};

struct Arena {
    char* base = nullptr;
    size_t off = 0, peak = 0, cap = 0;
    bool dry = false, overflow = false;
    void* alloc(size_t bytes) {
        off = align_up(off, 256);
        void* p = dry ? (void*)(uintptr_t)(0x1000 + off) : (void*)(base + off);
        off += bytes;
        if (off > peak) peak = off;
        if (!dry && off > cap) overflow = true;
        return p;
    }
    size_t mark() const { return off; }
    void release(size_t m) { off = m; }
};

struct UvTab { int w, h, C; float* tx; float* ty; };

struct ShapeTabs {
    int frames = 0;
    int* pos = nullptr;
    float *rope_cos = nullptr, *rope_sin = nullptr;
    int rope_npos = 0;
    const float* dino_pos = nullptr;
    std::vector<UvTab> uv;
    std::vector<void*> owned;
    ~ShapeTabs() {
        for (void* p : owned) (void)hipFree(p);
    }
};

#define TRACK_PART 1
#include "track_impl.inc"
#undef TRACK_PART

}

struct skimi_vggt {
    skimi_vggt_config cfg;
    std::map<std::string, std::pair<float*, int64_t>> raw;
    std::vector<void*> owned;
    bool finalized = false;
    bool dpt_fold = true;
    Lin patch_proj;
    int patch_kp = 0;
    float* dino_pos = nullptr;
    std::map<std::pair<int, int>, float*> dino_pos_alt;
    float* dino_special = nullptr;
    float* agg_special = nullptr;
    std::vector<BlockW> dino, frame, global;
    LNw dino_norm;
    CamW cam;
    DptW depth, point, trackf;
    TrackW track;
    std::mutex prep_mu;
    std::map<std::pair<int, int>, std::vector<std::unique_ptr<ShapeTabs>>> tabs;
};

namespace {

struct Packer {
    skimi_vggt* h;
    int rc = SKIMI_OK;
    hipStream_t st = nullptr;

    float* raw(const std::string& key, int64_t n) {
        if (rc) return nullptr;
        auto it = h->raw.find(key);
        if (it == h->raw.end()) {
            set_error("skimi_vggt_finalize: missing weight '%s'", key.c_str());
            rc = SKIMI_ERR_STATE;
            return nullptr;
        }
        if (it->second.second != n) {
            set_error("skimi_vggt_finalize: weight '%s' has %ld elements, expected %ld", key.c_str(),
                      (long)it->second.second, (long)n);
            rc = SKIMI_ERR_STATE;
            return nullptr;
        }
        return it->second.first;
    }
    void* dmalloc(size_t bytes) {
        if (rc) return nullptr;
        void* p = nullptr;
        if (hipMalloc(&p, bytes) != hipSuccess) {
            set_error("skimi_vggt_finalize: hipMalloc(%zu) failed", bytes);
            rc = SKIMI_ERR_HIP;
            return nullptr;
        }
        h->owned.push_back(p);
        return p;
    }
    float* keep(const std::string& key, int64_t n) {
        float* src = raw(key, n);
        if (!src) return nullptr;
        float* dst = (float*)dmalloc(n * 4);
        if (dst && hipMemcpyAsync(dst, src, n * 4, hipMemcpyDeviceToDevice, st) != hipSuccess) rc = SKIMI_ERR_HIP;
        return dst;
    }
    LNw ln(const std::string& p, int C) { return LNw{keep(p + ".weight", C), keep(p + ".bias", C)}; }

    Lin pack_matrix(float* src, int N, int K, int prec) {
        Lin L;
        L.N = N;
        L.K = (int)align_up((size_t)K, 8);
        L.prec = prec;
        if (rc) return L;
        float* m = src;
        if (L.K != K) {
            m = (float*)dmalloc((size_t)N * L.K * 4);
            if (m && (rc = pad_cols_launch(src, m, N, K, L.K, st))) return L;
        }
        if (prec == SKIMI_PREC_BF16 || prec == SKIMI_PREC_F16) {
            void* b = dmalloc((size_t)N * L.K * 2);
            if (b) rc = prec == SKIMI_PREC_F16 ? f32_to_f16_launch(m, b, (long)N * L.K, st) : f32_to_bf16_launch(m, b, (long)N * L.K, st);
            L.w = b;
            L.wdt = prec == SKIMI_PREC_F16 ? SKIMI_F16 : SKIMI_BF16;
        } else {
            if (m == src) {
                m = (float*)dmalloc((size_t)N * L.K * 4);
                if (m && hipMemcpyAsync(m, src, (size_t)N * L.K * 4, hipMemcpyDeviceToDevice, st) != hipSuccess)
                    rc = SKIMI_ERR_HIP;
            }
            L.w = m;
            L.wdt = SKIMI_F32;
        }
// ... 138 lines not shown
            if (f.has_r1) {
                f.r1c1 = conv(rp + ".resConfUnit1.conv1", features, features, 3, 1, 1, prec, true);
                f.r1c2 = conv(rp + ".resConfUnit1.conv2", features, features, 3, 1, 1, prec, true);
            }
            f.r2c1 = conv(rp + ".resConfUnit2.conv1", features, features, 3, 1, 1, prec, true);
            f.r2c2 = conv(rp + ".resConfUnit2.conv2", features, features, 3, 1, 1, prec, true);
        }
        if (feature_only) {
            d.oc1 = conv(p + ".scratch.output_conv1", features, features, 3, 1, 1, prec, true);
        } else {
            d.oc1 = conv(p + ".scratch.output_conv1", features / 2, features, 3, 1, 1, prec, true);
            d.oc2a = conv(p + ".scratch.output_conv2.0", 32, features / 2, 3, 1, 1, prec, true);
            if (!rc && prec == SKIMI_PREC_BF16X3 && (features / 2) % 32 == 0) {
                const int Ci = features / 2;
                float* src = raw(p + ".scratch.output_conv2.0.weight", (int64_t)32 * Ci * 9);
                d.oc2a_direct = (unsigned short*)dmalloc((size_t)32 * Ci * 9 * 2 * 2);
                if (!rc && d.oc2a_direct) rc = conv_direct_pack_launch(src, d.oc2a_direct, Ci, st);
                if (!rc && hipStreamSynchronize(st) != hipSuccess) rc = SKIMI_ERR_HIP;
            }
            d.oc2b_w = keep(p + ".scratch.output_conv2.2.weight", (int64_t)n_out * 32);
            d.oc2b_b = keep(p + ".scratch.output_conv2.2.bias", n_out);
        }
        return d;
    }
};

struct Ctx {
    skimi_vggt* h;
    hipStream_t st;
    const ShapeTabs* tabs = nullptr;
    Arena ar;
    int rc = SKIMI_OK;
    void* slab = nullptr;
    size_t slab_bytes = 0;

    bool dry() const { return ar.dry; }
    static int act_dt(int prec) { return prec == SKIMI_PREC_BF16X3 ? SKIMI_F32 : prec == SKIMI_PREC_F16 ? SKIMI_F16 : SKIMI_BF16; }
    static size_t esz(int dt) { return dt == SKIMI_F32 ? 4 : 2; }

    void gemm(skimi_gemm_desc& d) {
        const size_t mk = ar.mark();
        if (d.W_split != nullptr && d.a_dtype != SKIMI_BF16X3_REC) {
            d.x3_scratch_bytes = gemm_x3dma_scratch_bytes(&d);
            d.x3_scratch = ar.alloc(d.x3_scratch_bytes);
        }
        if (!rc && !dry()) rc = gemm_dispatch(&d, st, slab, slab_bytes, 0);
        ar.release(mk);
    }
    skimi_gemm_desc desc(const Lin& L, const void* A, int a_dt, long lda, int M, void* out, int out_dt, long ldo) {
        skimi_gemm_desc d;
        memset(&d, 0, sizeof d);
        d.M = M; d.N = L.N; d.K = L.K;
        d.A = A; d.a_dtype = a_dt; d.lda = lda;
        d.W = L.w; d.w_dtype = L.wdt; d.ldw = L.K;
        d.prec = L.prec;
        d.splitk_scratch_zeroed = 1;
        d.W_split = L.w_split;
        d.bias = L.b;
        d.out = out; d.out_dtype = out_dt; d.ldo = ldo;
        return d;
    }
    void conv_geom(skimi_gemm_desc& d, const ConvW& c, int N, int H, int W, int OH, int OW) {
        if (c.k == 1 && c.stride == 1) return;
        d.a_mode = c.kmode;
        d.cN = N; d.cH = H; d.cW = W; d.cC = c.cin; d.KH = c.k; d.KW = c.k;
        d.stride = c.stride; d.pad = c.pad; d.dil = 1; d.OH = OH; d.OW = OW;
    }
    void ln(const float* x, const float* x2, long ldx, long rows, int C, const LNw& w, float eps, void* out, int odt,
            long grp_rows = 0, long grp_stride = 0, long grp_off = 0) {
        if (rc || dry()) return;
        rc = layernorm_launch(x, x2, ldx, rows, C, w.g, w.b, eps, out, odt, C, st, grp_rows, grp_stride, grp_off);
    }
    void copy(void* dst, const void* src, size_t bytes) {
        if (rc || dry()) return;
        if (hipMemcpyAsync(dst, src, bytes, hipMemcpyDeviceToDevice, st) != hipSuccess) {
            set_error("hipMemcpyAsync failed");
            rc = SKIMI_ERR_HIP;
        }
    }
};

struct BlockBufs { void* xn; void* qkv; void* ao; void* hid; void* q8 = nullptr; void* q8s = nullptr; };

void run_block(Ctx& c, const BlockW& w, float* x, int batch, int seq, int C, int heads, float eps, bool rope,
               const BlockBufs& b) {
    const int M = batch * seq;
    const int prec = w.qkv.prec;
    const int adt = Ctx::act_dt(prec);
    const int qdt = adt == SKIMI_F16 ? SKIMI_BF16 : adt;
    const int hidden = w.fc1.N;
    const bool fp8 = w.qkv.wq != nullptr && b.q8 != nullptr;
    const bool ln_mx = fp8 && C % 256 == 0;
    const bool hid_mx = fp8 && gemm_fp8_mx_output_ok(M, hidden);
    const bool ao_mx = fp8 && w.proj.wq != nullptr && attention_mx_output_ok(qdt, heads, C / heads);
    auto as_records = [&](skimi_gemm_desc d, void* rec, size_t rec_bytes) {
        d.A = rec; d.a_dtype = SKIMI_BF16X3_REC;
        d.x3_scratch = (char*)rec + rec_bytes; d.x3_scratch_bytes = 256;
        return d;
    };
    const bool x3 = adt == SKIMI_F32 && C % 256 == 0;
    auto d_qkv = c.desc(w.qkv, b.xn, adt, C, M, b.qkv, qdt, 3 * C);
    bool rec_qkv = false;
    if (x3) {
        const auto q = as_records(d_qkv, b.xn, (size_t)M * C * 4);
        if ((rec_qkv = gemm_x3dma_eligible(&q))) d_qkv = q;
    }
    if (ln_mx) {
        if (!c.rc && !c.dry()) c.rc = layernorm_mx_launch(x, C, M, C, w.n1.g, w.n1.b, eps, b.q8, b.q8s, c.st);
    } else {
        c.ln(x, nullptr, C, M, C, w.n1, eps, b.xn, rec_qkv ? SKIMI_BF16X3_REC : adt);
    }
    if (fp8) {
        if (!ln_mx && !c.rc && !c.dry()) c.rc = quant_mx_launch(b.xn, SKIMI_BF16, C, M, C, b.q8, b.q8s, c.st);
        if (!c.rc && !c.dry())
            c.rc = gemm_fp8_launch(b.q8, b.q8s, w.qkv.wq, w.qkv.wq_scales, M, 3 * C, C, w.qkv.b, SKIMI_ACT_NONE, nullptr, nullptr, 0,
                                   b.qkv, SKIMI_BF16, 3 * C, c.st);
    } else {
        c.gemm(d_qkv);
    }
    int q_scaled = 0;
    if (!c.rc && !c.dry() && (w.qn_w || rope)) {
        const float q_scale = (1.0f / sqrtf((float)(C / heads))) * 1.44269504088896340736f;
        c.rc = qknorm_rope_launch(b.qkv, qdt, M, heads, w.qn_w, w.qn_b, w.kn_w, w.kn_b, 1e-5f, rope ? c.tabs->pos : nullptr,
                                  c.tabs->rope_cos, c.tabs->rope_sin, c.tabs->rope_npos, c.st, q_scale,
                                  qdt == SKIMI_BF16 && C / heads == 64 ? &q_scaled : nullptr);
    }
    auto d_proj = c.desc(w.proj, b.ao, adt, C, M, x, SKIMI_F32, C);
    d_proj.gamma = w.ls1; d_proj.resid = x; d_proj.ldr = C;
    int ao_rec = 0;
    if (x3 && C / heads == 64) {
        const auto q = as_records(d_proj, b.ao, (size_t)M * C * 4);
        ao_rec = gemm_x3dma_eligible(&q) ? 1 : 0;
    }
    if (!c.rc && !c.dry())
        c.rc = attention_launch(b.qkv, b.ao, qdt, batch, seq, heads, C / heads, c.st, q_scaled, adt == SKIMI_F32 ? b.hid : nullptr,
                                adt == SKIMI_F32 ? (size_t)M * hidden * 4 : 0, &ao_rec, adt == SKIMI_F16,
                                ao_mx ? b.q8 : nullptr, ao_mx ? b.q8s : nullptr);
    if (ao_rec && !c.dry()) d_proj = as_records(d_proj, b.ao, (size_t)M * C * 4);
    if (fp8 && w.proj.wq) {
        if (!ao_mx && !c.rc && !c.dry()) c.rc = quant_mx_launch(b.ao, SKIMI_BF16, C, M, C, b.q8, b.q8s, c.st);
        if (!c.rc && !c.dry())
            c.rc = gemm_fp8_launch(b.q8, b.q8s, w.proj.wq, w.proj.wq_scales, M, C, C, w.proj.b, SKIMI_ACT_NONE, w.ls1, x, C, x,
                                   SKIMI_F32, C, c.st);
    } else {
        c.gemm(d_proj);
    }
    auto d_fc1 = c.desc(w.fc1, b.xn, adt, C, M, b.hid, adt, hidden);
    d_fc1.act = SKIMI_ACT_GELU;
    auto d_fc2 = c.desc(w.fc2, b.hid, adt, hidden, M, x, SKIMI_F32, C);
    d_fc2.gamma = w.ls2; d_fc2.resid = x; d_fc2.ldr = C;
    bool rec_fc1 = false;
    if (x3) {
        const auto q1 = as_records(d_fc1, b.xn, (size_t)M * C * 4);
        if ((rec_fc1 = gemm_x3dma_eligible(&q1))) d_fc1 = q1;
        const auto q2 = as_records(d_fc2, b.hid, (size_t)M * hidden * 4);
        if (hidden % 32 == 0 && gemm_x3dma_eligible(&q2)) {
            d_fc2 = q2;
            d_fc1.out = nullptr;
            d_fc1.out_records = b.hid;
        }
    }
    if (ln_mx) {
        if (!c.rc && !c.dry()) c.rc = layernorm_mx_launch(x, C, M, C, w.n2.g, w.n2.b, eps, b.q8, b.q8s, c.st);
    } else {
        c.ln(x, nullptr, C, M, C, w.n2, eps, b.xn, rec_fc1 ? SKIMI_BF16X3_REC : adt);
    }
    if (fp8) {
        if (!ln_mx && !c.rc && !c.dry()) c.rc = quant_mx_launch(b.xn, SKIMI_BF16, C, M, C, b.q8, b.q8s, c.st);
        unsigned char* hq = (unsigned char*)b.hid;
        unsigned char* hs = hq + (size_t)M * hidden;
        if (hid_mx) {
            if (!c.rc && !c.dry())
                c.rc = gemm_fp8_launch(b.q8, b.q8s, w.fc1.wq, w.fc1.wq_scales, M, hidden, C, w.fc1.b, SKIMI_ACT_GELU, nullptr, nullptr, 0,
                                       hq, SKIMI_FP8MX, hidden, c.st, hs);
        } else {
            if (!c.rc && !c.dry())
                c.rc = gemm_fp8_launch(b.q8, b.q8s, w.fc1.wq, w.fc1.wq_scales, M, hidden, C, w.fc1.b, SKIMI_ACT_GELU, nullptr, nullptr, 0,
                                       b.hid, SKIMI_BF16, hidden, c.st);
            if (!c.rc && !c.dry()) c.rc = quant_mx_launch(b.hid, SKIMI_BF16, hidden, M, hidden, b.q8, b.q8s, c.st);
            hq = (unsigned char*)b.q8;
            hs = (unsigned char*)b.q8s;
        }
        if (!c.rc && !c.dry())
            c.rc = gemm_fp8_launch(hq, hs, w.fc2.wq, w.fc2.wq_scales, M, C, hidden, w.fc2.b, SKIMI_ACT_NONE, w.ls2, x, C, x,
                                   SKIMI_F32, C, c.st);
        return;
    }
    c.gemm(d_fc1);
    c.gemm(d_fc2);
}

const UvTab* find_uv(const ShapeTabs* h, int w, int hh, int C) {
    if (!h) return nullptr;
    for (const auto& t : h->uv)
        if (t.w == w && t.h == hh && t.C == C) return &t;
    return nullptr;
}

bool dpt_fused_ln(const DptW& w, int f2, int udt) {
    static const bool off = getenv("SKIMI_TRACK_LN_FUSED") && !atoi(getenv("SKIMI_TRACK_LN_FUSED"));
    return !off && w.feature_only && w.out_ln != nullptr && w.out_ln->g != nullptr && w.out_ln->b != nullptr && f2 == 128 && udt == SKIMI_F32;
}

void* run_dpt(Ctx& c, const DptW& w, float* const* sf, float* const* sg, int F, int P, int nsp, int ph, int pw, int C,
              int H, int W, float* pts, float* conf, int act_mode) {
    const int prec = w.proj[0].prec;
    const int adt = Ctx::act_dt(prec);
    const size_t es = Ctx::esz(adt);
    const int D = 2 * C, np = ph * pw, feat = w.features;
    const size_t mk = c.ar.mark();
    int hh[4] = {ph * 4, ph * 2, ph, (ph - 1) / 2 + 1};
    int ww[4] = {pw * 4, pw * 2, pw, (pw - 1) / 2 + 1};
    void* rn[4];
    for (int i = 0; i < 4; ++i) rn[i] = c.ar.alloc((size_t)F * hh[i] * ww[i] * feat * es);
    auto rec_bytes = [&](int lvl) { return (size_t)F * hh[lvl] * ww[lvl] * feat * 4 + 256; };
    auto takes_records = [&](const Lin& L, const ConvW* cw, int lvl) {
        if (adt != SKIMI_F32 || feat % 32 != 0 || L.w_split == nullptr) return false;
        char* fake = (char*)(uintptr_t)0x10000000;
        auto d = c.desc(L, fake, SKIMI_BF16X3_REC, feat, F * hh[lvl] * ww[lvl], fake, adt, L.N);
        if (cw) c.conv_geom(d, *cw, F, hh[lvl], ww[lvl], hh[lvl], ww[lvl]);
        d.x3_scratch = fake + rec_bytes(lvl) - 256;
        d.x3_scratch_bytes = 256;
        return gemm_x3dma_eligible(&d);
    };
    bool use_rec[4];
    char* rn_rec[4] = {nullptr, nullptr, nullptr, nullptr};
    for (int i = 0; i < 4; ++i) {
        use_rec[i] = takes_records(w.ref[i].r2c1.lin, &w.ref[i].r2c1, i);
        if (use_rec[i]) rn_rec[i] = (char*)c.ar.alloc(rec_bytes(i));
    }
    {
        const size_t mk2 = c.ar.mark();
        void* lnb = c.ar.alloc((size_t)F * np * D * es);
        void* lnb_rec = adt == SKIMI_F32 ? c.ar.alloc((size_t)F * np * D * 4 + 256) : nullptr;
        for (int i = 0; i < 4; ++i) {
            const size_t mk3 = c.ar.mark();
            void* t0 = c.ar.alloc((size_t)F * np * w.oc[i] * es);
            {
                auto d = c.desc(w.proj[i], lnb, adt, D, F * np, t0, adt, w.oc[i]);
                bool rec_in = false;
                if (adt == SKIMI_F32 && D % 256 == 0 && w.proj[i].w_split != nullptr) {
                    auto q = d;
                    q.a_dtype = SKIMI_BF16X3_REC;
                    q.x3_scratch = (char*)lnb_rec + (size_t)F * np * D * 4;
                    q.x3_scratch_bytes = 256;
                    q.A = lnb_rec;
                    rec_in = gemm_x3dma_eligible(&q);
                    if (rec_in) d = q;
                }
                c.ln(sf[i], sg[i], C, (long)F * np, D, w.norm, 1e-5f, rec_in ? lnb_rec : lnb, rec_in ? SKIMI_BF16X3_REC : adt, np, P, nsp);
                c.gemm(d);
            }
            if (i < 2 && adt == SKIMI_F32 && w.fold[i].w_split != nullptr) {
                const size_t t0_bytes = (size_t)F * np * w.oc[i] * 4;
                char* fake = (char*)(uintptr_t)0x10000000;
                auto d = c.desc(w.fold[i], fake, SKIMI_BF16X3_REC, w.oc[i], F * np, fake, adt, feat);
                d.a_mode = 3; d.store_mode = 2; d.ps_s = i == 0 ? 4 : 2; d.ps_C = feat;
                d.cN = F; d.cH = ph; d.cW = pw; d.cC = w.oc[i];
                d.x3_scratch = fake + t0_bytes; d.x3_scratch_bytes = 256;
                d.act = SKIMI_ACT_RELU;
                if (gemm_x3dma_eligible(&d)) {
                    char* t0_rec = (char*)c.ar.alloc(t0_bytes + 256);
                    const UvTab* t = w.pos_embed ? find_uv(c.tabs, pw, ph, w.oc[i]) : nullptr;
                    if (w.pos_embed && !t && !c.rc && !c.dry()) { set_error("uv table missing"); c.rc = SKIMI_ERR_STATE; }
                    if (!c.rc && !c.dry())
                        c.rc = add_uv_pos_records_launch((const float*)t0, t ? t->tx : nullptr, t ? t->ty : nullptr, F, ph, pw, w.oc[i],
                                                         t0_rec, c.st);
// ... 129 lines not shown
        d.x3_scratch = prev_rec + (size_t)F * h1 * w1 * feat * 4;
        d.x3_scratch_bytes = 256;
        if (!c.rc && !c.dry()) c.rc = gemm_dispatch(&d, c.st, c.slab, c.slab_bytes, 0);
    } else {
        auto d = c.desc(w.oc1.lin, prev, adt, feat, F * h1 * w1, c1, adt, f2);
        c.conv_geom(d, w.oc1, F, h1, w1, h1, w1);
        c.gemm(d);
    }
    const int Ho = ph * c.h->cfg.patch_size / w.down_ratio, Wo = pw * c.h->cfg.patch_size / w.down_ratio;
    const UvTab* uvt = w.pos_embed ? find_uv(c.tabs, Wo, Ho, f2) : nullptr;
    if (w.pos_embed && !uvt && !c.rc && !c.dry()) { set_error("uv table missing"); c.rc = SKIMI_ERR_STATE; }
    static const int no_direct = getenv("SKIMI_CONV_DIRECT") ? !atoi(getenv("SKIMI_CONV_DIRECT")) : 0;
    const bool direct = !w.feature_only && w.oc2a_direct != nullptr && adt == SKIMI_F32 && !no_direct;
    void* c2 = nullptr;
    if (direct) {
        const size_t pe = (size_t)F * Ho * Wo * f2;
        unsigned short* rec = (unsigned short*)c.ar.alloc(pe * 4);
        c2 = c.ar.alloc((size_t)F * Ho * Wo * 32 * es);
        if (!c.rc && !c.dry())
            c.rc = bilinear_ac_planes_launch((const float*)c1, rec, F, h1, w1, Ho, Wo, f2, c.st, uvt ? uvt->tx : nullptr,
                                             uvt ? uvt->ty : nullptr);
        if (!c.rc && !c.dry())
            c.rc = conv_direct_n32_launch(rec, rec + f2, w.oc2a_direct, w.oc2a.lin.b, (float*)c2, F, Ho, Wo, f2, 1, c.st,
                                          2L * f2);
    } else {
        const int udt = (w.feature_only && w.out_f32) ? SKIMI_F32 : adt;
        void* c1u = c.ar.alloc((size_t)F * Ho * Wo * f2 * Ctx::esz(udt));
        if (!c.rc && !c.dry())
            c.rc = dpt_fused_ln(w, f2, udt)
                       ? bilinear_ac_launch(c1, c1u, adt, F, h1, w1, Ho, Wo, f2, c.st, uvt ? uvt->tx : nullptr, uvt ? uvt->ty : nullptr, udt,
                                            w.out_ln->g, w.out_ln->b, 1e-5f)
                       : bilinear_ac_launch(c1, c1u, adt, F, h1, w1, Ho, Wo, f2, c.st, uvt ? uvt->tx : nullptr, uvt ? uvt->ty : nullptr, udt);
        if (w.feature_only) return c1u;
        c2 = c.ar.alloc((size_t)F * Ho * Wo * 32 * es);
        auto d = c.desc(w.oc2a.lin, c1u, adt, f2, F * Ho * Wo, c2, adt, 32);
        c.conv_geom(d, w.oc2a, F, Ho, Wo, Ho, Wo);
        d.act = SKIMI_ACT_RELU;
        c.gemm(d);
    }
    if (!c.rc && !c.dry())
        c.rc = dpt_out_launch(c2, adt, w.oc2b_w, w.oc2b_b, w.n_out, pts, conf, (long)F * Ho * Wo, act_mode, c.st);
    c.ar.release(mk);
    (void)H; (void)W;
    return nullptr;
}

#define TRACK_PART 2
#include "track_impl.inc"
#undef TRACK_PART

void run_camera(Ctx& c, const CamW& w, const float* sf, const float* sg, int B, int S, int P, int C, float* out_list,
                float* out_last) {
    const skimi_vggt_config& cfg = c.h->cfg;
    const int R = B * S, D = 2 * C;
    const size_t mk = c.ar.mark();
    float* pose_tokens = (float*)c.ar.alloc((size_t)R * D * 4);
    float* xn = (float*)c.ar.alloc((size_t)R * D * 4);
    float* xc = (float*)c.ar.alloc((size_t)R * D * 4);
    float* e = (float*)c.ar.alloc((size_t)R * D * 4);
    float* mod = (float*)c.ar.alloc((size_t)R * 3 * D * 4);
    float* pred16 = (float*)c.ar.alloc((size_t)R * 16 * 4);
    float* t2 = (float*)c.ar.alloc((size_t)R * (D / 2) * 4);
    float* delta = (float*)c.ar.alloc((size_t)R * 9 * 4);
    BlockBufs bb;
    bb.xn = c.ar.alloc((size_t)R * D * 4 + 256);
    bb.qkv = c.ar.alloc((size_t)R * 3 * D * 4);
    bb.ao = c.ar.alloc((size_t)R * D * 4 + 256);
    bb.hid = c.ar.alloc((size_t)R * 4 * D * 4 + 256);
    c.ln(sf, sg, (long)P * C, R, D, w.token_norm, 1e-5f, pose_tokens, SKIMI_F32);
    LNw none;
    for (int it = 0; it < cfg.cam_iters; ++it) {
        if (it == 0 && !c.rc && !c.dry()) c.rc = tile_vec_launch(w.empty16, pred16, 16, R, c.st);
        {
            auto d = c.desc(w.embed_pose, pred16, SKIMI_F32, 16, R, e, SKIMI_F32, D);
            d.act = SKIMI_ACT_SILU;
            c.gemm(d);
        }
        {
            auto d = c.desc(w.poseLN, e, SKIMI_F32, D, R, mod, SKIMI_F32, 3 * D);
            c.gemm(d);
        }
        c.ln(pose_tokens, nullptr, D, R, D, none, 1e-6f, xn, SKIMI_F32);
        if (!c.rc && !c.dry()) c.rc = adaln_launch(xn, pose_tokens, mod, xc, R, D, c.st);
        for (const BlockW& b : w.trunk) run_block(c, b, xc, B, S, D, cfg.cam_heads, 1e-5f, false, bb);
        c.ln(xc, nullptr, D, R, D, w.trunk_norm, 1e-5f, xn, SKIMI_F32);
        {
            auto d = c.desc(w.fc1, xn, SKIMI_F32, D, R, t2, SKIMI_F32, D / 2);
            d.act = SKIMI_ACT_GELU;
            c.gemm(d);
        }
        {
            auto d = c.desc(w.fc2, t2, SKIMI_F32, D / 2, R, delta, SKIMI_F32, 9);
            c.gemm(d);
        }
        float* dst = out_list ? out_list + (size_t)it * R * 9 : (it == cfg.cam_iters - 1 ? out_last : xn );
        if (!c.rc && !c.dry()) c.rc = pose_update_launch(delta, pred16, dst, R, it == 0, c.st);
        if (it == cfg.cam_iters - 1 && out_list && out_last) c.copy(out_last, dst, (size_t)R * 9 * 4);
    }
    c.ar.release(mk);
}

int prepare(skimi_vggt* h, int F, int S, int H, int W, const ShapeTabs** out) {
    auto& entries = h->tabs[std::make_pair(H, W)];
    int largest = 0;
    for (const auto& e : entries) {
        if (e->frames >= F) {
            *out = e.get();
            return SKIMI_OK;
        }
        largest = std::max(largest, e->frames);
    }
    const ShapeTabs* first = entries.empty() ? nullptr : entries.front().get();
    const int cap = std::max(F, 2 * largest);
    (void)S;
    std::unique_ptr<ShapeTabs> tabs(new ShapeTabs());
    ShapeTabs* t_ = tabs.get();
    t_->frames = cap;
    const skimi_vggt_config& cfg = h->cfg;
    const int p = cfg.patch_size, ph = H / p, pw = W / p, nsp = 1 + cfg.num_register_tokens, P = nsp + ph * pw;
    auto up = [&](const void* src, size_t bytes, void** dst) -> int {
        SKIMI_HIP(hipMalloc(dst, bytes));
        t_->owned.push_back(*dst);
        SKIMI_HIP(hipMemcpy(*dst, src, bytes, hipMemcpyHostToDevice));
        return SKIMI_OK;
    };
    int rc;
    if (cfg.use_dino) {
        const bool native = H == W && H == cfg.dino_img_size;
        t_->dino_pos = native ? h->dino_pos : h->dino_pos_alt.at({H, W});
    }
    std::vector<int> pos((size_t)cap * P * 2, 0);
    for (int f = 0; f < cap; ++f)
        for (int y = 0; y < ph; ++y)
            for (int x = 0; x < pw; ++x) {
                const size_t i = ((size_t)f * P + nsp + (size_t)y * pw + x) * 2;
                pos[i] = y + 1;
                pos[i + 1] = x + 1;
            }
    if ((rc = up(pos.data(), pos.size() * 4, (void**)&t_->pos))) return rc;
    if (first) {
        t_->rope_cos = first->rope_cos; t_->rope_sin = first->rope_sin; t_->rope_npos = first->rope_npos;
        t_->uv = first->uv;
        *out = t_;
        entries.push_back(std::move(tabs));
        return SKIMI_OK;
    }
    const int npos = std::max(ph, pw) + 1;
    std::vector<float> cs((size_t)npos * 16), sn((size_t)npos * 16);
    for (int i = 0; i < 16; ++i) {
        const float expo = (float)(2 * i) / 32.0f;
        const float inv = 1.0f / powf(100.0f, expo);
        for (int q = 0; q < npos; ++q) {
            const float a = (float)q * inv;
            cs[(size_t)q * 16 + i] = cosf(a);
            sn[(size_t)q * 16 + i] = sinf(a);
        }
    }
    if ((rc = up(cs.data(), cs.size() * 4, (void**)&t_->rope_cos))) return rc;
    if ((rc = up(sn.data(), sn.size() * 4, (void**)&t_->rope_sin))) return rc;
    t_->rope_npos = npos;
    auto add_uv = [&](int w, int hh, int C) -> int {
        if (find_uv(t_, w, hh, C)) return SKIMI_OK;
        const double aspect = (double)W / (double)H;
        const double diag = sqrt(aspect * aspect + 1.0);
        const double sx = aspect / diag, sy = 1.0 / diag;
        const int half = C / 2, quarter = C / 4;
        std::vector<float> tx((size_t)w * half), ty((size_t)hh * half);
// ... 3 lines not shown
            for (int i = 0; i < n; ++i) {
                const float pv = i < n / 2 ? lo + step * (float)i : hi - step * (float)(n - 1 - i);
                for (int j = 0; j < quarter; ++j) {
                    const double omega = 1.0 / pow(100.0, (double)j / (double)quarter);
                    const double a = (double)pv * omega;
                    tab[(size_t)i * half + j] = (float)sin(a) * 0.1f;
                    tab[(size_t)i * half + quarter + j] = (float)cos(a) * 0.1f;
                }
            }
        };
        fill(tx, w, sx);
        fill(ty, hh, sy);
        UvTab t{w, hh, C, nullptr, nullptr};
        int r2;
        if ((r2 = up(tx.data(), tx.size() * 4, (void**)&t.tx))) return r2;
        if ((r2 = up(ty.data(), ty.size() * 4, (void**)&t.ty))) return r2;
        t_->uv.push_back(t);
        return SKIMI_OK;
    };
    if (cfg.enable_depth || cfg.enable_point) {
        for (int i = 0; i < 4; ++i)
            if ((rc = add_uv(pw, ph, cfg.dpt_out_channels[i]))) return rc;
        if ((rc = add_uv(pw * p, ph * p, cfg.dpt_features / 2))) return rc;
    }
    *out = t_;
    entries.push_back(std::move(tabs));
    return SKIMI_OK;
}

int forward_impl(skimi_vggt* h, Ctx& c, const float* images, const float* query, int B, int S, int H, int W, int nq,
                 const skimi_vggt_outputs* out) {
    const skimi_vggt_config& cfg = h->cfg;
    const int p = cfg.patch_size, C = cfg.embed_dim, ph = H / p, pw = W / p, np = ph * pw;
    const int nsp = 1 + cfg.num_register_tokens, P = nsp + np, F = B * S, M = F * P;
    const int prec = cfg.prec, adt = Ctx::act_dt(prec);
    const size_t es = Ctx::esz(adt);

    c.slab_bytes = std::max<size_t>((size_t)F * 6 * C * 4 * 4 * 4, 4u << 20);
    c.slab = c.ar.alloc(c.slab_bytes);
    if (!c.dry() && hipMemsetAsync(c.slab, 0, c.slab_bytes, c.st) != hipSuccess) c.rc = SKIMI_ERR_HIP;

    float* x = (float*)c.ar.alloc((size_t)M * C * 4);
    std::vector<int> keep;
    auto want = [&](int l) { for (int k : keep) if (k == l) return; keep.push_back(l); };
    const bool run_depth = cfg.enable_depth && out && (out->depth || out->depth_conf);
    const bool run_point = cfg.enable_point && out && (out->world_points || out->world_points_conf);
    const bool run_cam = cfg.enable_camera && out && (out->pose_enc || out->pose_enc_list);
    const bool do_track = cfg.enable_track && out && out->track && query && nq > 0;
    if (run_depth || run_point || do_track) for (int i = 0; i < 4; ++i) want(cfg.dpt_layers[i]);
    if (run_cam || (out && out->tokens_last)) want(cfg.depth - 1);
    std::map<int, std::pair<float*, float*>> saved;
    for (int l : keep) {
        float* a = (float*)c.ar.alloc((size_t)M * C * 4);
        float* b = (float*)c.ar.alloc((size_t)M * C * 4);
        saved[l] = {a, b};
    }
    {
        const size_t mk = c.ar.mark();
        BlockBufs bb;
        bb.xn = c.ar.alloc((size_t)M * C * es + 256);
        bb.qkv = c.ar.alloc((size_t)M * 3 * C * es);
        bb.ao = c.ar.alloc((size_t)M * C * es + 256);
        bb.hid = c.ar.alloc((size_t)M * 4 * C * es + 256);
        if (cfg.prec == SKIMI_PREC_FP8) {
            const size_t kp = align_up((size_t)4 * C, 128);
            bb.q8 = c.ar.alloc((size_t)M * kp);
            bb.q8s = c.ar.alloc((size_t)M * (kp / 32));
        }
        void* pa = c.ar.alloc((size_t)F * np * h->patch_kp * es);
        if (!c.rc && !c.dry()) c.rc = patch_gather_launch(images, pa, adt, F, H, W, p, h->patch_kp, c.st);
        {
            auto d = c.desc(h->patch_proj, pa, adt, h->patch_kp, F * np, x, SKIMI_F32, C);
            d.out_rows_per_batch = np; d.out_batch_stride = P; d.out_row_off = nsp;
            if (cfg.use_dino) {
                const bool native = H == W && H == cfg.dino_img_size;
                (void)native;
                d.resid = c.tabs ? c.tabs->dino_pos : h->dino_pos; d.ldr = C;
                d.resid_rows_per_batch = np; d.resid_batch_stride = 0; d.resid_row_off = 1;
            }
            c.gemm(d);
        }
        if (cfg.use_dino) {
            if (!c.rc && !c.dry()) c.rc = special_tokens_launch(x, h->dino_special, F, S, P, nsp, C, c.st);
            for (const BlockW& b : h->dino) run_block(c, b, x, F, P, C, cfg.dino_heads, 1e-6f, false, bb);
            c.ln(x, nullptr, C, M, C, h->dino_norm, 1e-6f, x, SKIMI_F32);
        }
        if (!c.rc && !c.dry()) c.rc = special_tokens_launch(x, h->agg_special, F, S, P, nsp, C, c.st);
        for (int i = 0; i < cfg.depth && !c.rc; ++i) {
            run_block(c, h->frame[i], x, F, P, C, cfg.num_heads, 1e-5f, true, bb);
            auto it = saved.find(i);
            if (it != saved.end()) c.copy(it->second.first, x, (size_t)M * C * 4);
            run_block(c, h->global[i], x, B, S * P, C, cfg.num_heads, 1e-5f, true, bb);
            if (it != saved.end()) c.copy(it->second.second, x, (size_t)M * C * 4);
        }
        c.ar.release(mk);
    }
    if (out && out->tokens_last && !c.rc && !c.dry()) {
        auto& sv = saved[cfg.depth - 1];
        if (hipMemcpy2DAsync(out->tokens_last, (size_t)2 * C * 4, sv.first, (size_t)C * 4, (size_t)C * 4, M,
                             hipMemcpyDeviceToDevice, c.st) != hipSuccess ||
            hipMemcpy2DAsync(out->tokens_last + C, (size_t)2 * C * 4, sv.second, (size_t)C * 4, (size_t)C * 4, M,
                             hipMemcpyDeviceToDevice, c.st) != hipSuccess) {
            set_error("hipMemcpy2DAsync failed");
            c.rc = SKIMI_ERR_HIP;
        }
    }
    if (run_cam) {
        auto& sv = saved[cfg.depth - 1];
        run_camera(c, h->cam, sv.first, sv.second, B, S, P, C, out->pose_enc_list, out->pose_enc);
    }
    float* sf[4];
    float* sg[4];
    if (run_depth || run_point || do_track)
        for (int i = 0; i < 4; ++i) {
            sf[i] = saved[cfg.dpt_layers[i]].first;
            sg[i] = saved[cfg.dpt_layers[i]].second;
        }
    if (run_depth) {
        float* pts = out->depth ? out->depth : (float*)c.ar.alloc((size_t)F * H * W * 4);
        float* cf = out->depth_conf ? out->depth_conf : (float*)c.ar.alloc((size_t)F * H * W * 4);
        run_dpt(c, h->depth, sf, sg, F, P, nsp, ph, pw, C, H, W, pts, cf, 0);
    }
    if (run_point) {
        float* pts = out->world_points ? out->world_points : (float*)c.ar.alloc((size_t)F * H * W * 3 * 4);
        float* cf = out->world_points_conf ? out->world_points_conf : (float*)c.ar.alloc((size_t)F * H * W * 4);
        run_dpt(c, h->point, sf, sg, F, P, nsp, ph, pw, C, H, W, pts, cf, 1);
    }
    if (do_track) run_track(c, sf, sg, B, S, P, nsp, ph, pw, C, H, W, query, nq, out->track, out->vis, out->conf);
    return c.rc;
}

}

extern "C" {

skimi_vggt* skimi_vggt_create(const skimi_vggt_config* cfg) {
    if (!cfg) { set_error("skimi_vggt_create: null config"); return nullptr; }
    if (cfg->embed_dim <= 0 || cfg->num_heads <= 0 || cfg->embed_dim / cfg->num_heads != 64 ||
        cfg->embed_dim % cfg->num_heads != 0) {
        set_error("skimi_vggt_create: embed_dim / num_heads must be 64");
        return nullptr;
    }
    if (cfg->use_dino && cfg->embed_dim / cfg->dino_heads != 64) {
        set_error("skimi_vggt_create: DINOv2 head_dim must be 64");
        return nullptr;
    }
    if (cfg->patch_size <= 0 || cfg->depth <= 0 || cfg->num_register_tokens < 0) {
        set_error("skimi_vggt_create: bad sizes");
        return nullptr;
    }
    for (int i = 0; i < 4; ++i)
        if (cfg->dpt_layers[i] < 0 || cfg->dpt_layers[i] >= cfg->depth) {
            set_error("skimi_vggt_create: dpt_layers[%d] = %d outside [0, depth)", i, cfg->dpt_layers[i]);
            return nullptr;
        }
    if (cfg->prec < SKIMI_PREC_BF16 || cfg->prec > SKIMI_PREC_F16) {
        set_error("skimi_vggt_create: prec %d is not one of SKIMI_PREC_BF16 / BF16X3 / FP8 / F16", cfg->prec);
        return nullptr;
    }
    if (cfg->head_prec != SKIMI_PREC_BF16 && cfg->head_prec != SKIMI_PREC_BF16X3 && cfg->head_prec != SKIMI_PREC_F16) {
        set_error("skimi_vggt_create: head_prec %d: the depth / point heads run in SKIMI_PREC_BF16X3 (the reference's fp32) or, as a "
                  "faster, less accurate option, on SKIMI_PREC_F16 / SKIMI_PREC_BF16 operands", cfg->head_prec);
        return nullptr;
    }
    skimi_vggt* h = new skimi_vggt();
    h->cfg = *cfg;
    h->dpt_fold = !(getenv("SKIMI_DPT_FOLD") && atoi(getenv("SKIMI_DPT_FOLD")) == 0);
    return h;
}

void skimi_vggt_destroy(skimi_vggt* h) {
    if (!h) return;
    for (auto& kv : h->raw) (void)hipFree(kv.second.first);
    for (void* p : h->owned) (void)hipFree(p);
    h->tabs.clear();
    for (auto& kv : h->dino_pos_alt) (void)hipFree(kv.second);
    delete h;
}

int skimi_vggt_set_weight(skimi_vggt* h, const char* key, const float* data, int64_t n, int32_t on_device) {
    SKIMI_CHECK_ARG(h && key && data && n > 0, "skimi_vggt_set_weight: bad arguments");
    float* d = nullptr;
    SKIMI_HIP(hipMalloc((void**)&d, (size_t)n * 4));
    hipError_t e = hipMemcpy(d, data, (size_t)n * 4, on_device ? hipMemcpyDeviceToDevice : hipMemcpyHostToDevice);
    if (e != hipSuccess) {
        (void)hipFree(d);
        set_error("skimi_vggt_set_weight: copy failed: %s", hipGetErrorString(e));
        return SKIMI_ERR_HIP;
    }
    auto it = h->raw.find(key);
    if (it != h->raw.end()) (void)hipFree(it->second.first);
    h->raw[key] = {d, n};
    h->finalized = false;
    return SKIMI_OK;
}

int skimi_vggt_set_pos_embed(skimi_vggt* h, int32_t H, int32_t W, const float* pos_embed, int32_t on_device) {
    SKIMI_CHECK_ARG(h && pos_embed && h->cfg.use_dino, "skimi_vggt_set_pos_embed: needs a DINOv2 model and a table");
    const int p = h->cfg.patch_size;
    SKIMI_CHECK_ARG(H > 0 && W > 0 && H % p == 0 && W % p == 0, "skimi_vggt_set_pos_embed: bad size %dx%d", H, W);
    const size_t n = ((size_t)(H / p) * (W / p) + 1) * h->cfg.embed_dim;
    float* d = nullptr;
    SKIMI_HIP(hipMalloc((void**)&d, n * 4));
    hipError_t e = hipMemcpy(d, pos_embed, n * 4, on_device ? hipMemcpyDeviceToDevice : hipMemcpyHostToDevice);
    if (e != hipSuccess) {
        (void)hipFree(d);
        set_error("skimi_vggt_set_pos_embed: copy failed: %s", hipGetErrorString(e));
        return SKIMI_ERR_HIP;
    }
    std::lock_guard<std::mutex> lk(h->prep_mu);
    auto it = h->dino_pos_alt.find({H, W});
    if (it != h->dino_pos_alt.end()) {
        e = hipMemcpy(it->second, d, n * 4, hipMemcpyDeviceToDevice);
        (void)hipFree(d);
        if (e != hipSuccess) {
            set_error("skimi_vggt_set_pos_embed: copy failed: %s", hipGetErrorString(e));
            return SKIMI_ERR_HIP;
        }
        return SKIMI_OK;
    }
    h->dino_pos_alt[{H, W}] = d;
    return SKIMI_OK;
}

int skimi_vggt_finalize(skimi_vggt* h) {
    SKIMI_CHECK_ARG(h, "skimi_vggt_finalize: null handle");
    const skimi_vggt_config& cfg = h->cfg;
    for (void* p : h->owned) (void)hipFree(p);
    h->owned.clear();
    Packer pk{h};
    const int C = cfg.embed_dim, p = cfg.patch_size, R = cfg.num_register_tokens, nsp = 1 + R;
    const int hidden = 4 * C, D = 2 * C;
    const std::string A = "aggregator";
    const int kraw = 3 * p * p;
    const std::string pe = cfg.use_dino ? A + ".patch_embed.patch_embed.proj" : A + ".patch_embed.proj";
    h->patch_proj = pk.linear(pe, C, kraw, cfg.prec == SKIMI_PREC_FP8 ? SKIMI_PREC_BF16 : cfg.prec);
    h->patch_kp = h->patch_proj.K;
    if (cfg.use_dino) {
        const std::string d = A + ".patch_embed";
        const int g = cfg.dino_img_size / p, np0 = g * g;
        h->dino_pos = pk.keep(d + ".pos_embed", (int64_t)(np0 + 1) * C);
        float* cls = pk.raw(d + ".cls_token", C);
        float* reg = R ? pk.raw(d + ".register_tokens", (int64_t)R * C) : nullptr;
        (void)pk.raw(d + ".mask_token", C);
        h->dino_special = (float*)pk.dmalloc((size_t)2 * nsp * C * 4);
        if (!pk.rc) {
            std::vector<float> hc(C), hp(C), hr((size_t)R * C), tab((size_t)2 * nsp * C);
            SKIMI_HIP(hipMemcpy(hc.data(), cls, C * 4, hipMemcpyDeviceToHost));
            SKIMI_HIP(hipMemcpy(hp.data(), h->dino_pos, C * 4, hipMemcpyDeviceToHost));
            if (R) SKIMI_HIP(hipMemcpy(hr.data(), reg, (size_t)R * C * 4, hipMemcpyDeviceToHost));
// ... 134 lines not shown
```

skiing_analysis_pytorch_amd/ops.py:

```python
from __future__ import annotations

import ctypes as C
from typing import NamedTuple, Optional

import torch

from . import _lib
from ._lib import ACT_NONE, BF16, F16, F32, PREC_BF16, PREC_BF16X3, GemmDesc, check, lib, ptr


def _dt(t: torch.Tensor) -> int:
    if t.dtype == torch.float32:
        return F32
    if t.dtype == torch.bfloat16:
        return BF16
    if t.dtype == torch.float16:
        return F16
    raise TypeError(f"unsupported dtype {t.dtype}")


def _require_cuda(*ts):
    for t in ts:
        if t is not None and not t.is_cuda:
            raise _lib.SkimiError("libskimi ops need device (HBM) tensors; got a CPU tensor")


def gemm(a, w, *, prec=PREC_BF16X3, bias=None, gamma=None, resid=None, act=ACT_NONE, out=None,
         out_dtype=torch.float32, conv=None, resid_map=None, pixel_shuffle=None, splitk_scratch=None,
         force_splitk=0, M=None, lda=None, w_split=None, x3_scratch=None, a_records=None, out_records=None,
         records_only=False, post_act=ACT_NONE, resid2=None, out2=None, out_map=None, splitk_zeroed=False):
    _require_cuda(w, bias, gamma, resid, out, resid2, out2)
    if out_map is not None and out is None:
        raise _lib.SkimiError("gemm: out_map needs a caller-owned out (the remapped rows cannot be sized here)")
    if resid is not None and resid2 is not None and resid.dtype != resid2.dtype:
        raise _lib.SkimiError("gemm: resid and resid2 share one dtype (resid_dtype)")
    d = GemmDesc()
    N, K = w.shape
    d.N, d.K = N, K
    d.W, d.w_dtype = ptr(w), _dt(w)
    if a_records is not None:
        _require_cuda(a_records)
        d.A, d.a_dtype = ptr(a_records), _lib.BF16X3_REC
        d.lda = lda if lda is not None else (conv["C"] if conv is not None else K)
    else:
        _require_cuda(a)
        d.A, d.a_dtype = ptr(a), _dt(a)
        d.lda = lda if lda is not None else a.stride(-2) if a.dim() >= 2 else a.shape[-1]
    dev = w.device
    d.ldw = w.stride(0)
    d.prec = prec
    if conv is not None:
        d.a_mode = 2 if conv.get("slice_major") else 1
        d.cN, d.cH, d.cW, d.cC = conv["N"], conv["H"], conv["W"], conv["C"]
        d.KH, d.KW, d.stride, d.pad, d.dil = conv["KH"], conv["KW"], conv["stride"], conv["pad"], conv["dil"]
        d.OH, d.OW = conv["OH"], conv["OW"]
        d.M = d.cN * d.OH * d.OW
    else:
        d.M = M if M is not None else a.shape[0]
    if records_only:
        assert out is None and out_records is not None and pixel_shuffle is None
        d.out_dtype = _lib.F32
    elif pixel_shuffle is not None:
        s, cout, n_img, h, w_ = pixel_shuffle
        d.store_mode, d.ps_s, d.ps_C = 1, s, cout
        d.cN, d.cH, d.cW = n_img, h, w_
        if out is None:
            out = torch.empty((n_img, h * s, w_ * s, cout), dtype=out_dtype, device=dev)
        d.ldo = out.stride(-2)
    else:
        if out is None:
            out = torch.empty((d.M, N), dtype=out_dtype, device=dev)
        d.ldo = out.stride(-2)
    if not records_only:
        d.out, d.out_dtype = ptr(out), _dt(out)
    if out2 is not None:
        if out is None or (out2.dtype == torch.float32) == (out.dtype == torch.float32) or \
                (out.dtype == torch.float32 and out2.dtype != torch.bfloat16):
            raise _lib.SkimiError("gemm: out2 is the other dtype of out (bf16 next to fp32, fp32 next to 16-bit)")
        d.out2, d.ldo2 = ptr(out2), out2.stride(-2)
    if out_map is not None:
        d.out_rows_per_batch, d.out_batch_stride, d.out_row_off = out_map
    d.bias, d.gamma, d.resid = ptr(bias), ptr(gamma), ptr(resid)
    if resid is not None:
        d.ldr = resid.stride(-2)
        d.resid_dtype = _dt(resid)
    if resid2 is not None:
        d.resid2, d.ldr2 = ptr(resid2), resid2.stride(-2)
        d.resid_dtype = _dt(resid2)
    if resid_map is not None:
        d.resid_rows_per_batch, d.resid_batch_stride, d.resid_row_off = resid_map
    d.act = act
    d.post_act = post_act
    if splitk_scratch is not None:
        d.splitk_scratch = ptr(splitk_scratch)
        d.splitk_scratch_bytes = splitk_scratch.numel() * splitk_scratch.element_size()
    d.force_splitk = force_splitk
    d.splitk_scratch_zeroed = int(splitk_zeroed)
    if w_split is not None:
        d.W_split = ptr(w_split)
        if a_records is not None:
            d.x3_scratch = ptr(a_records) + a_records.numel() * 2 - 256
            d.x3_scratch_bytes = 256
        else:
            d.x3_scratch = ptr(x3_scratch)
            d.x3_scratch_bytes = x3_scratch.numel() * x3_scratch.element_size()
    if out_records is not None:
        _require_cuda(out_records)
        d.out_records = ptr(out_records)
    check(lib().skimi_gemm(C.byref(d), _lib.current_stream()), "skimi_gemm")
    return out


class GemmPath(NamedTuple):
    family: Optional[str]
    tile: Optional[str]
    loop: Optional[str]
    mfma: Optional[int]
    epi: int
    splitk: int
    raw: int


_PATH_FAMILY = {1: "generic", 2: "splitk_ordered", 3: "splitk_atomic", 4: "x3dma_wide", 5: "x3dma_narrow",
                6: "gemm256", 7: "conv_win"}
_PATH_TILE = {1: "64x64", 2: "128x64", 3: "128x128"}
_PATH_LOOP = {1: "two_phase_256", 2: "two_phase_192", 3: "ping_pong", 4: "single_stream"}


def gemm_last_path() -> GemmPath:
    v = int(lib().skimi_gemm_last_path())
    fam = _PATH_FAMILY.get(v & 15)
    sub = (v >> 4) & 15
    generic = fam in ("generic", "splitk_ordered", "splitk_atomic")
    return GemmPath(family=fam, tile=_PATH_TILE.get(sub) if generic else None,
                    loop=_PATH_LOOP.get(sub) if fam == "gemm256" else None,
                    mfma={1: 16, 2: 32}.get((v >> 8) & 15), epi=(v >> 12) & 15, splitk=(v >> 16) & 255, raw=v)


def layernorm(x, gamma=None, beta=None, eps=1e-5, *, x2=None, out_dtype=torch.float32):
    _require_cuda(x, x2, gamma, beta)
    rows = x.numel() // x.shape[-1]
    Cc = x.shape[-1] * (2 if x2 is not None else 1)
    out = torch.empty((*x.shape[:-1], Cc), dtype=out_dtype, device=x.device)
    check(lib().skimi_layernorm(ptr(x), ptr(x2), x.stride(-2), rows, Cc, ptr(gamma), ptr(beta), eps, ptr(out),
                                _dt(out), Cc, _lib.current_stream()), "skimi_layernorm")
    return out


def qknorm_rope_(qkv, heads, qn_w=None, qn_b=None, kn_w=None, kn_b=None, eps=1e-5, pos=None, rope_cos=None,
                 rope_sin=None, *, q_scale=None):
    _require_cuda(qkv, pos, rope_cos, rope_sin)
    tokens = qkv.numel() // (3 * heads * 64)
    npos = rope_cos.shape[0] if rope_cos is not None else 0
    if q_scale is not None:
        flag = C.c_int32(0)
        check(lib().skimi_qknorm_rope_scaled(ptr(qkv), _dt(qkv), tokens, heads, ptr(qn_w), ptr(qn_b), ptr(kn_w), ptr(kn_b),
                                             eps, ptr(pos), ptr(rope_cos), ptr(rope_sin), npos, q_scale, C.byref(flag),
                                             _lib.current_stream()), "skimi_qknorm_rope_scaled")
        return qkv, bool(flag.value)
    check(lib().skimi_qknorm_rope(ptr(qkv), _dt(qkv), tokens, heads, ptr(qn_w), ptr(qn_b), ptr(kn_w), ptr(kn_b),
                                  eps, ptr(pos), ptr(rope_cos), ptr(rope_sin), npos, _lib.current_stream()),
          "skimi_qknorm_rope")
    return qkv


def attention_x3_scratch_bytes(tokens, row_elems):
    return int(lib().skimi_attention_x3_scratch_bytes(tokens, row_elems))


def attention(qkv, batch, seq, heads, head_dim, out_dtype=None, *, q_prescaled=0, x3_scratch=None, out_records=False,
              out=None):
    _require_cuda(qkv)
    if q_prescaled or x3_scratch is not None or out_records or out is not None:
        return _attention_ex(qkv, batch, seq, heads, head_dim, out_dtype, q_prescaled, x3_scratch, out_records, out)
    if isinstance(out_dtype, str):
        assert out_dtype == "fp8mx", out_dtype
        rows, Kp = batch * seq, (heads * head_dim + 127) // 128 * 128
        buf = torch.zeros(rows * (Kp + Kp // 32), dtype=torch.uint8, device=qkv.device)
        check(lib().skimi_attention_out(ptr(qkv), ptr(buf), _dt(qkv), _lib.FP8MX, batch, seq, heads, head_dim,
                                        _lib.current_stream()), "skimi_attention_out")
        return buf[:rows * Kp].view(rows, Kp), buf[rows * Kp:].view(rows, Kp // 32)
    out = torch.empty((batch * seq, heads * head_dim), dtype=out_dtype or qkv.dtype, device=qkv.device)
    if out_dtype is None or out_dtype == qkv.dtype:
        check(lib().skimi_attention(ptr(qkv), ptr(out), _dt(qkv), batch, seq, heads, head_dim, _lib.current_stream()),
              "skimi_attention")
    else:
        check(lib().skimi_attention_out(ptr(qkv), ptr(out), _dt(qkv), _dt(out), batch, seq, heads, head_dim,
                                        _lib.current_stream()), "skimi_attention_out")
    return out


# ... 156 lines not shown
```

Baseline: 18.01.

## Fuse QK layernorm and RoPE into QKV GEMM epilogue; skip saved-layer copies

```diff
diff --git a/include/skimi.h b/include/skimi.h
--- a/include/skimi.h
+++ b/include/skimi.h
@@ -76,6 +76,18 @@
     void* x3_scratch;
     uint64_t x3_scratch_bytes;
     void* out_records;
+    int32_t qk_epilogue;
+    int32_t qk_heads;
+    const float* qn_w;
+    const float* qn_b;
+    const float* kn_w;
+    const float* kn_b;
+    const int32_t* qk_pos;
+    const float* rope_cos;
+    const float* rope_sin;
+    int32_t rope_npos;
+    float qk_eps;
+    float q_scale;
 } skimi_gemm_desc;
 
 int skimi_split_planes(const float* x, int64_t ld, int64_t rows, int32_t C, void* hi, void* lo, void* stream);
diff --git a/skiing_analysis_pytorch_amd/_lib.py b/skiing_analysis_pytorch_amd/_lib.py
--- a/skiing_analysis_pytorch_amd/_lib.py
+++ b/skiing_analysis_pytorch_amd/_lib.py
@@ -50,6 +50,10 @@
         ("force_splitk", C.c_int32), ("splitk_scratch_zeroed", C.c_int32),
         ("W_split", C.c_void_p), ("x3_scratch", C.c_void_p), ("x3_scratch_bytes", C.c_uint64),
         ("out_records", C.c_void_p),
+        ("qk_epilogue", C.c_int32), ("qk_heads", C.c_int32),
+        ("qn_w", C.c_void_p), ("qn_b", C.c_void_p), ("kn_w", C.c_void_p), ("kn_b", C.c_void_p),
+        ("qk_pos", C.c_void_p), ("rope_cos", C.c_void_p), ("rope_sin", C.c_void_p),
+        ("rope_npos", C.c_int32), ("qk_eps", C.c_float), ("q_scale", C.c_float),
     ]
 
 
diff --git a/skiing_analysis_pytorch_amd/csrc/gemm.hip b/skiing_analysis_pytorch_amd/csrc/gemm.hip
--- a/skiing_analysis_pytorch_amd/csrc/gemm.hip
+++ b/skiing_analysis_pytorch_amd/csrc/gemm.hip
@@ -423,6 +423,11 @@
     }
     if (d->resid) SKIMI_CHECK_ARG(d->ldr >= d->N, "skimi_gemm: ldr < N");
     if (d->resid2) SKIMI_CHECK_ARG(d->ldr2 >= d->N, "skimi_gemm: ldr2 < N");
+    if (d->qk_epilogue)
+        SKIMI_CHECK_ARG(force_splitk <= 0 && gemm_qk_epilogue_eligible(d),
+                        "skimi_gemm: qk_epilogue runs on the 256 x 256 LDS-DMA kernel only (16-bit operands, plain rows, M >= 2048, "
+                        "K %% 64 == 0, bias only, bf16 out with 16-byte aligned rows, N = 3 * qk_heads * 64, qk_heads * 64 %% 256 == 0, "
+                        "both norm weights, positions and tables, rope_npos <= 128)");
 
     GemmArgs a;
     a.M = d->M; a.N = d->N; a.K = d->K;
@@ -443,6 +448,12 @@
     a.partial = nullptr;
     a.f16 = d->prec == SKIMI_PREC_F16;
     a.splitk_ordered = 0;
+    if (d->qk_epilogue) {
+        a.qk_epi = 1; a.qk_heads = d->qk_heads;
+        a.qn_w = d->qn_w; a.qn_b = d->qn_b; a.kn_w = d->kn_w; a.kn_b = d->kn_b;
+        a.qk_pos = d->qk_pos; a.rope_cos = d->rope_cos; a.rope_sin = d->rope_sin; a.rope_npos = d->rope_npos;
+        a.qk_eps = d->qk_eps; a.q_scale = d->q_scale;
+    }
     {
         auto al16 = [](const void* q) { return ((uintptr_t)q & 15) == 0; };
         const bool out_ok = d->out_dtype == SKIMI_F32 ? al16(d->out) : (((uintptr_t)d->out & 7) == 0);
diff --git a/skiing_analysis_pytorch_amd/csrc/gemm256.hip b/skiing_analysis_pytorch_amd/csrc/gemm256.hip
--- a/skiing_analysis_pytorch_amd/csrc/gemm256.hip
+++ b/skiing_analysis_pytorch_amd/csrc/gemm256.hip
@@ -2,6 +2,7 @@
 
 #include "common.h"
 #include "gemm_epilogue.h"
+#include "qknorm_row.h"
 
 namespace skimi {
 
@@ -33,15 +34,15 @@
     return hb;
 }
 
-template <int MT>
+template <int MT, int P = 64>
 __device__ __forceinline__ void acc_to_slab(float* stg, const f32x16 (&acc)[MT][2], int i, int lane) {
     const int l31 = lane & 31, lh = lane >> 5;
 #pragma unroll
     for (int j = 0; j < 2; ++j)
 #pragma unroll
-        for (int r = 0; r < 16; ++r) stg[((r & 3) + 8 * (r >> 2) + 4 * lh) * 64 + j * 32 + l31] = acc[i][j][r];
-}
-template <int MT>
+        for (int r = 0; r < 16; ++r) stg[((r & 3) + 8 * (r >> 2) + 4 * lh) * P + j * 32 + l31] = acc[i][j][r];
+}
+template <int MT, int P = 64>
 __device__ __forceinline__ void acc_to_slab(float* stg, const f32x4 (&acc)[2 * MT][4], int i, int lane) {
     const int l15 = lane & 15, lq = lane >> 4;
 #pragma unroll
@@ -49,7 +50,98 @@
 #pragma unroll
         for (int c = 0; c < 4; ++c)
 #pragma unroll
-            for (int r = 0; r < 4; ++r) stg[(16 * b + 4 * lq + r) * 64 + 16 * c + l15] = acc[2 * i + b][c][r];
+            for (int r = 0; r < 4; ++r) stg[(16 * b + 4 * lq + r) * P + 16 * c + l15] = acc[2 * i + b][c][r];
+}
+
+constexpr int QK_PITCH = 68;
+constexpr int QK_TAB_OFF = 36 * 1024;
+constexpr int QK_TAB_MAX = 24 * 1024;
+
+struct QkTab { float c[8], s[8]; };
+__device__ __forceinline__ void qk_tables_load(const GemmArgs& p, QkTab& t, int tid, int n0) {
+    if (n0 >= 2 * p.qk_heads * 64) return;
+    const int last = p.rope_npos * 16 - 1;
+#pragma unroll
+    for (int k = 0; k < 8; ++k) {
+        const int i = min(tid + 256 * k, last);
+        t.c[k] = p.rope_cos[i];
+        t.s[k] = p.rope_sin[i];
+    }
+}
+__device__ __forceinline__ void qk_tables_store(const GemmArgs& p, const QkTab& t, char* smem, int tid, int n0) {
+    if (n0 >= 2 * p.qk_heads * 64) return;
+    float* tab = reinterpret_cast<float*>(smem + QK_TAB_OFF);
+    const int nt = p.rope_npos * 16;
+#pragma unroll
+    for (int k = 0; k < 8; ++k) {
+        const int i = min(tid + 256 * k, nt - 1);
+        tab[i] = t.c[k];
+        tab[nt + i] = t.s[k];
+        tab[2 * nt + i] = -t.s[k];
+    }
+    __syncthreads();
+}
+
+template <int MT, bool EDGE, typename ACC>
+__device__ __forceinline__ void epilogue256_qk_tile(const GemmArgs& p, ACC& acc, char* smem, int wave, int lane, int wr, int wc,
+                                                    int m0, int n0) {
+    constexpr int P = QK_PITCH;
+    float* stg = reinterpret_cast<float*>(smem) + wave * (32 * P);
+    const float* tab = reinterpret_cast<const float*>(smem + QK_TAB_OFF);
+    const int sub = lane & 7;
+    const bool is_q = n0 < p.qk_heads * 64;
+    const int n = n0 + wc * 64 + 8 * sub;
+    const float* nw = (is_q ? p.qn_w : p.kn_w) + 8 * sub;
+    const float* nb = is_q ? p.qn_b : p.kn_b;
+    float w[8], b[8], bs[8];
+#pragma unroll
+    for (int j = 0; j < 8; ++j) {
+        w[j] = nw[j];
+        b[j] = nb ? nb[8 * sub + j] : 0.f;
+        bs[j] = p.bias ? p.bias[n + j] : 0.f;
+    }
+    const int sect = sub >> 2;
+    const int d0 = (8 * sub) & 15;
+    const int npos = p.rope_npos;
+    const bool lower = ((8 * sub) & 31) < 16;
+    const int sin0 = (lower ? 2 : 1) * npos * 16 + d0;
+    const float scale = is_q ? p.q_scale : 1.f;
+    const int mrow0 = m0 + wr * (32 * MT) + (lane >> 3);
+    int pp[MT][4];
+#pragma unroll
+    for (int i = 0; i < MT; ++i)
+#pragma unroll
+        for (int it = 0; it < 4; ++it) {
+            int m = mrow0 + i * 32 + it * 8;
+            if (EDGE) m = min(m, p.M - 1);
+            pp[i][it] = p.qk_pos[2 * (long)m + sect];
+        }
+#pragma unroll
+    for (int i = 0; i < MT; ++i) {
+        acc_to_slab<MT, P>(stg, acc, i, lane);
+        __builtin_amdgcn_fence(__ATOMIC_RELEASE, "wavefront");
+        __builtin_amdgcn_s_waitcnt(0xC07F);
+#pragma unroll
+        for (int it = 0; it < 4; ++it) {
+            const float* row = &stg[(it * 8 + (lane >> 3)) * P + 8 * sub];
+            const float4 v0 = *reinterpret_cast<const float4*>(row), v1 = *reinterpret_cast<const float4*>(row + 4);
+            const int ps = min(max(pp[i][it], 0), npos - 1);
+            const float4 c0 = *reinterpret_cast<const float4*>(&tab[ps * 16 + d0]);
+            const float4 c1 = *reinterpret_cast<const float4*>(&tab[ps * 16 + d0 + 4]);
+            const float4 s0 = *reinterpret_cast<const float4*>(&tab[sin0 + ps * 16]);
+            const float4 s1 = *reinterpret_cast<const float4*>(&tab[sin0 + ps * 16 + 4]);
+            const float ct[8] = {c0.x, c0.y, c0.z, c0.w, c1.x, c1.y, c1.z, c1.w};
+            const float st[8] = {s0.x, s0.y, s0.z, s0.w, s1.x, s1.y, s1.z, s1.w};
+            const float v[8] = {v0.x, v0.y, v0.z, v0.w, v1.x, v1.y, v1.z, v1.w};
+            float t[8];
+#pragma unroll
+            for (int j = 0; j < 8; ++j) t[j] = bf2f(f2bf(v[j] + bs[j]));
+            const bf16x8 o = qknorm_rope_row8(t, w, b, p.qk_eps, ct, st, scale);
+            const int m = mrow0 + i * 32 + it * 8;
+            if (!EDGE || m < p.M) *reinterpret_cast<bf16x8*>((unsigned short*)p.out + (long)m * p.ldo + n) = o;
+        }
+        __builtin_amdgcn_s_waitcnt(0xC07F);
+    }
 }
 
 template <int MT, int EPI, int PF = 2, bool H16 = false, typename ACC>
@@ -59,6 +151,16 @@
     const int n = n0 + wc * 64 + 4 * (lane & 15);
     if (p.dbg & 8) {
         if (acc[0][0][0] == 123.456f) ((float*)p.out)[0] = acc[MT - 1][1][sizeof(acc[0][0]) / 4 - 1];
+        return;
+    }
+    if constexpr (EPI == 4) {
+        if (n0 >= 2 * p.qk_heads * 64) {
+            epilogue256<MT, 1, PF, false>(p, acc, smem, wave, lane, wr, wc, m0, n0);
+        } else if ((m0 + 64 * MT <= p.M) && !(p.dbg & 4)) {
+            epilogue256_qk_tile<MT, false>(p, acc, smem, wave, lane, wr, wc, m0, n0);
+        } else {
+            epilogue256_qk_tile<MT, true>(p, acc, smem, wave, lane, wr, wc, m0, n0);
+        }
         return;
     }
     const bool interior = (m0 + 64 * MT <= p.M) && (n0 + 256 <= p.N) && !(p.dbg & 4);
@@ -605,6 +707,8 @@
     SKIMI_W4_KTILE(false, false);
 #undef SKIMI_W4_KTILE
 #undef SKIMI_W4_HEAD
+    QkTab qtab;
+    if constexpr (EPI == 4) qk_tables_load(p, qtab, tid, n0);
     asm volatile("s_nop 7\n\ts_nop 4");
 #pragma unroll
     for (int h = 0; h < 2; ++h)
@@ -615,6 +719,7 @@
     __builtin_amdgcn_s_waitcnt(0xC07F);
     SKIMI_BAR();
 
+    if constexpr (EPI == 4) qk_tables_store(p, qtab, smem, tid, n0);
     epilogue256<4, EPI, 4, F16 && EPI == 3>(p, acc[0], smem, wave, lane, wr, 2 * wc, m0, n0);
     epilogue256<4, EPI, 4, F16 && EPI == 3>(p, acc[1], smem, wave, lane, wr, 2 * wc + 1, m0, n0);
     } else {
@@ -726,9 +831,12 @@
 #undef SKIMI_W4_HEAD
 #undef SKIMI_W4_TAIL
 #undef SKIMI_W4_MFMA
+    QkTab qtab;
+    if constexpr (EPI == 4) qk_tables_load(p, qtab, tid, n0);
     __builtin_amdgcn_s_waitcnt(0xC07F);
     SKIMI_BAR();
 
+    if constexpr (EPI == 4) qk_tables_store(p, qtab, smem, tid, n0);
     epilogue256<4, EPI, 4, F16 && EPI == 3>(p, acc[0], smem, wave, lane, wr, 2 * wc, m0, n0);
     epilogue256<4, EPI, 4, F16 && EPI == 3>(p, acc[1], smem, wave, lane, wr, 2 * wc + 1, m0, n0);
     }
@@ -948,6 +1056,18 @@
            d->N >= 512 && (((uintptr_t)d->A | (uintptr_t)d->W) & 15) == 0;
 }
 
+bool gemm_qk_epilogue_eligible(const skimi_gemm_desc* d) {
+    if (!gemm256_eligible(d)) return false;
+    const bool plain = d->out != nullptr && d->out_dtype == SKIMI_BF16 && d->out_rows_per_batch == 0 && d->out_row_off == 0 &&
+                       d->out2 == nullptr && d->out_records == nullptr && d->gamma == nullptr && d->resid == nullptr &&
+                       d->resid2 == nullptr && d->act == SKIMI_ACT_NONE && d->post_act == SKIMI_ACT_NONE &&
+                       ((uintptr_t)d->out & 15) == 0 && d->ldo % 8 == 0 && ((uintptr_t)d->bias & 15) == 0;
+    if (!plain) return false;
+    if (d->qk_heads <= 0 || (long)d->N != 3L * d->qk_heads * 64 || (d->qk_heads * 64) % 256 != 0) return false;
+    if (!d->qn_w || !d->kn_w || !d->qk_pos || !d->rope_cos || !d->rope_sin) return false;
+    return d->rope_npos > 0 && (size_t)d->rope_npos * 192 <= (size_t)QK_TAB_MAX;
+}
+
 template <int MT, int EPI, bool F16 = false>
 static int launch256(GemmArgs& a, hipStream_t st) {
     constexpr size_t lds = 2ull * (64 * MT + 256) * 128;
@@ -997,6 +1117,7 @@
         if (epi == 1) return launch256w4<1, F16, M16>(a, st);
         if (epi == 2) return launch256w4<2, F16, M16>(a, st);
         if (epi == 3) return launch256w4<3, F16, M16>(a, st);
+        if (epi == 4) return launch256w4<4, F16, M16>(a, st);
         return launch256w4<0, F16, M16>(a, st);
     }
     if (epi == 1) return launch256pp<1, F16, M16>(a, st);
@@ -1033,13 +1154,13 @@
         const long tiles = cdiv(a.M, bm) * cdiv(a.N, 256);
         return (double)cdiv(tiles, 256) * bm;
     };
-    const int epi = epi_kind(a);
+    const int epi = a.qk_epi ? 4 : epi_kind(a);
     const bool m16 = SKIMI_ENV_INT("SKIMI_GEMM256_MFMA", 16) != 32;
     const int use_pp = SKIMI_ENV_INT("SKIMI_GEMM256_PP", 1);
     const int use_mt3 = SKIMI_ENV_INT("SKIMI_GEMM256_MT3", -1);
     const int use_w4 = SKIMI_ENV_INT("SKIMI_GEMM256_W4", -1);
-    const bool mt3 = use_mt3 == 1 || (use_mt3 < 0 && cost(192) < 0.8 * cost(256));
-    const bool w4 = use_w4 >= 0 ? use_w4 != 0 : (epi == 1 || (epi == 2 && a.K > 1024));
+    const bool mt3 = epi != 4 && (use_mt3 == 1 || (use_mt3 < 0 && cost(192) < 0.8 * cost(256)));
+    const bool w4 = epi == 4 || (use_w4 >= 0 ? use_w4 != 0 : (epi == 1 || (epi == 2 && a.K > 1024)));
     const int loop = mt3 ? 2 : w4 ? 4 : (use_pp || a.f16) ? 3 : 1;
     set_gemm_path(SKIMI_GEMM_PATH_GEMM256, loop, (loop >= 3 && m16) ? 1 : 2, epi, 1);
     return a.f16 ? gemm256_pick<true>(a, st, epi, mt3, w4, use_pp, m16) : gemm256_pick<false>(a, st, epi, mt3, w4, use_pp, m16);
diff --git a/skiing_analysis_pytorch_amd/csrc/gemm_epilogue.h b/skiing_analysis_pytorch_amd/csrc/gemm_epilogue.h
--- a/skiing_analysis_pytorch_amd/csrc/gemm_epilogue.h
+++ b/skiing_analysis_pytorch_amd/csrc/gemm_epilogue.h
@@ -44,6 +44,18 @@
     const unsigned char* w_scales;
     long lsa, lsw;
     unsigned char* out_scales;
+    int qk_epi = 0;
+    int qk_heads = 0;
+    const float* qn_w = nullptr;
+    const float* qn_b = nullptr;
+    const float* kn_w = nullptr;
+    const float* kn_b = nullptr;
+    const int* qk_pos = nullptr;
+    const float* rope_cos = nullptr;
+    const float* rope_sin = nullptr;
+    int rope_npos = 0;
+    float qk_eps = 0.f;
+    float q_scale = 1.f;
 };
 
 __device__ __forceinline__ void store_rec4(const GemmArgs& p, long m, int n, float v0, float v1, float v2, float v3) {
@@ -246,6 +258,7 @@
 int gemm_last_path();
 
 bool gemm256_eligible(const skimi_gemm_desc* d);
+bool gemm_qk_epilogue_eligible(const skimi_gemm_desc* d);
 bool gemm_x3dma_eligible(const skimi_gemm_desc* d);
 int gemm_x3dma_launch(GemmArgs& a, const skimi_gemm_desc* d, hipStream_t st);
 size_t gemm_x3dma_scratch_bytes(const skimi_gemm_desc* d);
diff --git a/skiing_analysis_pytorch_amd/csrc/qknorm_row.h b/skiing_analysis_pytorch_amd/csrc/qknorm_row.h
--- /dev/null
+++ b/skiing_analysis_pytorch_amd/csrc/qknorm_row.h
@@ -0,0 +1,44 @@
+#pragma once
+#include "common.h"
+
+namespace skimi {
+
+__device__ __forceinline__ float dpp_xor1(float v) {
+    return __int_as_float(__builtin_amdgcn_update_dpp(0, __float_as_int(v), 0xB1, 0xF, 0xF, true));
+}
+__device__ __forceinline__ float dpp_xor2(float v) {
+    return __int_as_float(__builtin_amdgcn_update_dpp(0, __float_as_int(v), 0x4E, 0xF, 0xF, true));
+}
+__device__ __forceinline__ float dpp_mirror8(float v) {
+    return __int_as_float(__builtin_amdgcn_update_dpp(0, __float_as_int(v), 0x141, 0xF, 0xF, true));
+}
+__device__ __forceinline__ float sum8(float s) {
+    s += dpp_xor1(s);
+    s += dpp_xor2(s);
+    s += dpp_mirror8(s);
+    return s;
+}
+
+__device__ __forceinline__ bf16x8 qknorm_rope_row8(float (&t)[8], const float (&w)[8], const float (&b)[8], float eps,
+                                                   const float (&ct)[8], const float (&sst)[8], float scale) {
+    float s = 0.f;
+#pragma unroll
+    for (int j = 0; j < 8; ++j) s += t[j];
+    const float mean = sum8(s) * (1.f / 64.f);
+    float q = 0.f;
+#pragma unroll
+    for (int j = 0; j < 8; ++j) { t[j] -= mean; q += t[j] * t[j]; }
+    const float rstd = rsqrtf(sum8(q) * (1.f / 64.f) + eps);
+#pragma unroll
+    for (int j = 0; j < 8; ++j) t[j] = t[j] * rstd * w[j] + b[j];
+    bf16x8 o;
+#pragma unroll
+    for (int j = 0; j < 8; ++j) {
+        const float other = dpp_xor2(t[j]);
+        const float r = t[j] * ct[j] + other * sst[j];
+        o[j] = (short)f2bf(r * scale);
+    }
+    return o;
+}
+
+}
diff --git a/skiing_analysis_pytorch_amd/csrc/rowops.hip b/skiing_analysis_pytorch_amd/csrc/rowops.hip
--- a/skiing_analysis_pytorch_amd/csrc/rowops.hip
+++ b/skiing_analysis_pytorch_amd/csrc/rowops.hip
@@ -2,6 +2,7 @@
 
 #include "common.h"
 #include "kernels.h"
+#include "qknorm_row.h"
 
 namespace skimi {
 
@@ -302,22 +303,6 @@
     }
 }
 
-__device__ __forceinline__ float dpp_xor1(float v) {
-    return __int_as_float(__builtin_amdgcn_update_dpp(0, __float_as_int(v), 0xB1, 0xF, 0xF, true));
-}
-__device__ __forceinline__ float dpp_xor2(float v) {
-    return __int_as_float(__builtin_amdgcn_update_dpp(0, __float_as_int(v), 0x4E, 0xF, 0xF, true));
-}
-__device__ __forceinline__ float dpp_mirror8(float v) {
-    return __int_as_float(__builtin_amdgcn_update_dpp(0, __float_as_int(v), 0x141, 0xF, 0xF, true));
-}
-__device__ __forceinline__ float sum8(float s) {
-    s += dpp_xor1(s);
-    s += dpp_xor2(s);
-    s += dpp_mirror8(s);
-    return s;
-}
-
 __global__ __launch_bounds__(256) void qknorm_rope_bf16_kernel(unsigned short* __restrict__ qkv, long tokens, int heads,
                                                                const float* __restrict__ qn_w,
                                                                const float* __restrict__ qn_b,
@@ -328,8 +313,10 @@
                                                                const float* __restrict__ rsin, int npos, float q_scale) {
     extern __shared__ __attribute__((aligned(16))) float tab[];
     for (int i = threadIdx.x; i < npos * 16; i += 256) {
+        const float sn = rsin[i];
         tab[i] = rcos[i];
-        tab[npos * 16 + i] = rsin[i];
+        tab[npos * 16 + i] = sn;
+        tab[2 * npos * 16 + i] = -sn;
     }
     __syncthreads();
     const int sub = threadIdx.x & 7;
@@ -342,6 +329,7 @@
     const int sect = sub >> 2;
     const int d0 = (8 * sub) & 15;
     const bool lower = ((8 * sub) & 31) < 16;
+    const int sin0 = (lower ? 2 : 1) * npos * 16 + d0;
     const long total = tokens * heads;
     const long step = (long)gridDim.x * 32;
     const long trips = (total + step - 1) / step;
@@ -358,8 +346,8 @@
         pp = min(max(pp, 0), npos - 1);
         const float4 c0 = *reinterpret_cast<const float4*>(&tab[pp * 16 + d0]);
         const float4 c1 = *reinterpret_cast<const float4*>(&tab[pp * 16 + d0 + 4]);
-        const float4 s0 = *reinterpret_cast<const float4*>(&tab[npos * 16 + pp * 16 + d0]);
-        const float4 s1 = *reinterpret_cast<const float4*>(&tab[npos * 16 + pp * 16 + d0 + 4]);
+        const float4 s0 = *reinterpret_cast<const float4*>(&tab[sin0 + pp * 16]);
+        const float4 s1 = *reinterpret_cast<const float4*>(&tab[sin0 + pp * 16 + 4]);
         const float ct[8] = {c0.x, c0.y, c0.z, c0.w, c1.x, c1.y, c1.z, c1.w};
         const float st[8] = {s0.x, s0.y, s0.z, s0.w, s1.x, s1.y, s1.z, s1.w};
         bf16x8 outv[2];
@@ -368,23 +356,7 @@
             float t[8];
 #pragma unroll
             for (int j = 0; j < 8; ++j) t[j] = bf2f((unsigned short)raw[z][j]);
-            float s = 0.f;
-#pragma unroll
-            for (int j = 0; j < 8; ++j) s += t[j];
-            const float mean = sum8(s) * (1.f / 64.f);
-            float q = 0.f;
-#pragma unroll
-            for (int j = 0; j < 8; ++j) { t[j] -= mean; q += t[j] * t[j]; }
-            const float rstd = rsqrtf(sum8(q) * (1.f / 64.f) + eps);
-#pragma unroll
-            for (int j = 0; j < 8; ++j) t[j] = t[j] * rstd * w[z][j] + b[z][j];
-#pragma unroll
-            for (int j = 0; j < 8; ++j) {
-                const float other = dpp_xor2(t[j]);
-                const float rot = lower ? -other : other;
-                const float r = t[j] * ct[j] + rot * st[j];
-                outv[z][j] = (short)f2bf(z == 0 ? r * q_scale : r);
-            }
+            outv[z] = qknorm_rope_row8(t, w[z], b[z], eps, ct, st, z == 0 ? q_scale : 1.f);
         }
         if (live) {
             *reinterpret_cast<bf16x8*>(pq) = outv[0];
@@ -401,9 +373,10 @@
     if (q_scaled) *q_scaled = 0;
     SKIMI_CHECK_ARG(pos == nullptr || (rope_cos && rope_sin && rope_npos > 0), "skimi_qknorm_rope: pos without tables");
     if (((uintptr_t)qkv & 15) == 0 && dtype == SKIMI_BF16 && qn_w && kn_w && pos && rope_npos * 128 <= 48 * 1024) {
+        SKIMI_LDS_OPT_IN(qknorm_rope_bf16_kernel, 72 * 1024, "qknorm_rope_bf16");
         const long total = tokens * heads;
         const unsigned blocks = (unsigned)std::min<long>(cdiv(total, 32), 256 * 8);
-        hipLaunchKernelGGL(qknorm_rope_bf16_kernel, dim3(blocks), dim3(256), (size_t)rope_npos * 128, st,
+        hipLaunchKernelGGL(qknorm_rope_bf16_kernel, dim3(blocks), dim3(256), (size_t)rope_npos * 192, st,
                            (unsigned short*)qkv, (long)tokens, heads, qn_w, qn_b, kn_w, kn_b, eps, pos, rope_cos, rope_sin,
                            rope_npos, q_scaled ? q_scale : 1.f);
         if (q_scaled) *q_scaled = 1;
diff --git a/skiing_analysis_pytorch_amd/csrc/vggt.hip b/skiing_analysis_pytorch_amd/csrc/vggt.hip
--- a/skiing_analysis_pytorch_amd/csrc/vggt.hip
+++ b/skiing_analysis_pytorch_amd/csrc/vggt.hip
@@ -107,6 +107,8 @@
     std::vector<void*> owned;
     bool finalized = false;
     bool dpt_fold = true;
+    bool keep_copy = false;
+    bool qkv_fused = true;
     Lin patch_proj;
     int patch_kp = 0;
     float* dino_pos = nullptr;
@@ -411,8 +413,8 @@
 
 struct BlockBufs { void* xn; void* qkv; void* ao; void* hid; void* q8 = nullptr; void* q8s = nullptr; };
 
-void run_block(Ctx& c, const BlockW& w, float* x, int batch, int seq, int C, int heads, float eps, bool rope,
-               const BlockBufs& b) {
+void run_block(Ctx& c, const BlockW& w, const float* x_in, float* x_mid, float* x_out, int batch, int seq, int C, int heads,
+               float eps, bool rope, const BlockBufs& b) {
     const int M = batch * seq;
     const int prec = w.qkv.prec;
     const int adt = Ctx::act_dt(prec);
@@ -435,9 +437,19 @@
         if ((rec_qkv = gemm_x3dma_eligible(&q))) d_qkv = q;
     }
     if (ln_mx) {
-        if (!c.rc && !c.dry()) c.rc = layernorm_mx_launch(x, C, M, C, w.n1.g, w.n1.b, eps, b.q8, b.q8s, c.st);
+        if (!c.rc && !c.dry()) c.rc = layernorm_mx_launch(x_in, C, M, C, w.n1.g, w.n1.b, eps, b.q8, b.q8s, c.st);
     } else {
-        c.ln(x, nullptr, C, M, C, w.n1, eps, b.xn, rec_qkv ? SKIMI_BF16X3_REC : adt);
+        c.ln(x_in, nullptr, C, M, C, w.n1, eps, b.xn, rec_qkv ? SKIMI_BF16X3_REC : adt);
+    }
+    const float q_scale = (1.0f / sqrtf((float)(C / heads))) * 1.44269504088896340736f;
+    bool qk_fused = false;
+    if (!fp8 && !c.dry() && c.h && c.h->qkv_fused && rope && w.qn_w && w.kn_w && qdt == SKIMI_BF16 && C / heads == 64) {
+        auto q = d_qkv;
+        q.qk_epilogue = 1; q.qk_heads = heads;
+        q.qn_w = w.qn_w; q.qn_b = w.qn_b; q.kn_w = w.kn_w; q.kn_b = w.kn_b;
+        q.qk_pos = c.tabs->pos; q.rope_cos = c.tabs->rope_cos; q.rope_sin = c.tabs->rope_sin; q.rope_npos = c.tabs->rope_npos;
+        q.qk_eps = 1e-5f; q.q_scale = q_scale;
+        if ((qk_fused = gemm_qk_epilogue_eligible(&q))) d_qkv = q;
     }
     if (fp8) {
         if (!ln_mx && !c.rc && !c.dry()) c.rc = quant_mx_launch(b.xn, SKIMI_BF16, C, M, C, b.q8, b.q8s, c.st);
@@ -447,15 +459,14 @@
     } else {
         c.gemm(d_qkv);
     }
-    int q_scaled = 0;
-    if (!c.rc && !c.dry() && (w.qn_w || rope)) {
-        const float q_scale = (1.0f / sqrtf((float)(C / heads))) * 1.44269504088896340736f;
+    int q_scaled = qk_fused ? 1 : 0;
+    if (!qk_fused && !c.rc && !c.dry() && (w.qn_w || rope)) {
         c.rc = qknorm_rope_launch(b.qkv, qdt, M, heads, w.qn_w, w.qn_b, w.kn_w, w.kn_b, 1e-5f, rope ? c.tabs->pos : nullptr,
                                   c.tabs->rope_cos, c.tabs->rope_sin, c.tabs->rope_npos, c.st, q_scale,
                                   qdt == SKIMI_BF16 && C / heads == 64 ? &q_scaled : nullptr);
     }
-    auto d_proj = c.desc(w.proj, b.ao, adt, C, M, x, SKIMI_F32, C);
-    d_proj.gamma = w.ls1; d_proj.resid = x; d_proj.ldr = C;
+    auto d_proj = c.desc(w.proj, b.ao, adt, C, M, x_mid, SKIMI_F32, C);
+    d_proj.gamma = w.ls1; d_proj.resid = x_in; d_proj.ldr = C;
     int ao_rec = 0;
     if (x3 && C / heads == 64) {
         const auto q = as_records(d_proj, b.ao, (size_t)M * C * 4);
@@ -469,15 +480,15 @@
     if (fp8 && w.proj.wq) {
         if (!ao_mx && !c.rc && !c.dry()) c.rc = quant_mx_launch(b.ao, SKIMI_BF16, C, M, C, b.q8, b.q8s, c.st);
         if (!c.rc && !c.dry())
-            c.rc = gemm_fp8_launch(b.q8, b.q8s, w.proj.wq, w.proj.wq_scales, M, C, C, w.proj.b, SKIMI_ACT_NONE, w.ls1, x, C, x,
+            c.rc = gemm_fp8_launch(b.q8, b.q8s, w.proj.wq, w.proj.wq_scales, M, C, C, w.proj.b, SKIMI_ACT_NONE, w.ls1, x_in, C, x_mid,
                                    SKIMI_F32, C, c.st);
     } else {
         c.gemm(d_proj);
     }
     auto d_fc1 = c.desc(w.fc1, b.xn, adt, C, M, b.hid, adt, hidden);
     d_fc1.act = SKIMI_ACT_GELU;
-    auto d_fc2 = c.desc(w.fc2, b.hid, adt, hidden, M, x, SKIMI_F32, C);
-    d_fc2.gamma = w.ls2; d_fc2.resid = x; d_fc2.ldr = C;
+    auto d_fc2 = c.desc(w.fc2, b.hid, adt, hidden, M, x_out, SKIMI_F32, C);
+    d_fc2.gamma = w.ls2; d_fc2.resid = x_mid; d_fc2.ldr = C;
     bool rec_fc1 = false;
     if (x3) {
         const auto q1 = as_records(d_fc1, b.xn, (size_t)M * C * 4);
@@ -490,9 +501,9 @@
         }
     }
     if (ln_mx) {
-        if (!c.rc && !c.dry()) c.rc = layernorm_mx_launch(x, C, M, C, w.n2.g, w.n2.b, eps, b.q8, b.q8s, c.st);
+        if (!c.rc && !c.dry()) c.rc = layernorm_mx_launch(x_mid, C, M, C, w.n2.g, w.n2.b, eps, b.q8, b.q8s, c.st);
     } else {
-        c.ln(x, nullptr, C, M, C, w.n2, eps, b.xn, rec_fc1 ? SKIMI_BF16X3_REC : adt);
+        c.ln(x_mid, nullptr, C, M, C, w.n2, eps, b.xn, rec_fc1 ? SKIMI_BF16X3_REC : adt);
     }
     if (fp8) {
         if (!ln_mx && !c.rc && !c.dry()) c.rc = quant_mx_launch(b.xn, SKIMI_BF16, C, M, C, b.q8, b.q8s, c.st);
@@ -511,7 +522,7 @@
             hs = (unsigned char*)b.q8s;
         }
         if (!c.rc && !c.dry())
-            c.rc = gemm_fp8_launch(hq, hs, w.fc2.wq, w.fc2.wq_scales, M, C, hidden, w.fc2.b, SKIMI_ACT_NONE, w.ls2, x, C, x,
+            c.rc = gemm_fp8_launch(hq, hs, w.fc2.wq, w.fc2.wq_scales, M, C, hidden, w.fc2.b, SKIMI_ACT_NONE, w.ls2, x_mid, C, x_out,
                                    SKIMI_F32, C, c.st);
         return;
     }
@@ -807,7 +818,7 @@
         }
         c.ln(pose_tokens, nullptr, D, R, D, none, 1e-6f, xn, SKIMI_F32);
         if (!c.rc && !c.dry()) c.rc = adaln_launch(xn, pose_tokens, mod, xc, R, D, c.st);
-        for (const BlockW& b : w.trunk) run_block(c, b, xc, B, S, D, cfg.cam_heads, 1e-5f, false, bb);
+        for (const BlockW& b : w.trunk) run_block(c, b, xc, xc, xc, B, S, D, cfg.cam_heads, 1e-5f, false, bb);
         c.ln(xc, nullptr, D, R, D, w.trunk_norm, 1e-5f, xn, SKIMI_F32);
         {
             auto d = c.desc(w.fc1, xn, SKIMI_F32, D, R, t2, SKIMI_F32, D / 2);
@@ -977,16 +988,22 @@
         }
         if (cfg.use_dino) {
             if (!c.rc && !c.dry()) c.rc = special_tokens_launch(x, h->dino_special, F, S, P, nsp, C, c.st);
-            for (const BlockW& b : h->dino) run_block(c, b, x, F, P, C, cfg.dino_heads, 1e-6f, false, bb);
+            for (const BlockW& b : h->dino) run_block(c, b, x, x, x, F, P, C, cfg.dino_heads, 1e-6f, false, bb);
             c.ln(x, nullptr, C, M, C, h->dino_norm, 1e-6f, x, SKIMI_F32);
         }
         if (!c.rc && !c.dry()) c.rc = special_tokens_launch(x, h->agg_special, F, S, P, nsp, C, c.st);
+        const bool keep_copy = h->keep_copy;
+        const float* cur = x;
         for (int i = 0; i < cfg.depth && !c.rc; ++i) {
-            run_block(c, h->frame[i], x, F, P, C, cfg.num_heads, 1e-5f, true, bb);
             auto it = saved.find(i);
-            if (it != saved.end()) c.copy(it->second.first, x, (size_t)M * C * 4);
-            run_block(c, h->global[i], x, B, S * P, C, cfg.num_heads, 1e-5f, true, bb);
-            if (it != saved.end()) c.copy(it->second.second, x, (size_t)M * C * 4);
+            const bool direct = it != saved.end() && !keep_copy;
+            float* xf = direct ? it->second.first : x;
+            float* xg = direct ? it->second.second : x;
+            run_block(c, h->frame[i], cur, x, xf, F, P, C, cfg.num_heads, 1e-5f, true, bb);
+            if (it != saved.end() && !direct) c.copy(it->second.first, x, (size_t)M * C * 4);
+            run_block(c, h->global[i], xf, x, xg, B, S * P, C, cfg.num_heads, 1e-5f, true, bb);
+            if (it != saved.end() && !direct) c.copy(it->second.second, x, (size_t)M * C * 4);
+            cur = xg;
         }
         c.ar.release(mk);
     }
@@ -1061,6 +1078,8 @@
     skimi_vggt* h = new skimi_vggt();
     h->cfg = *cfg;
     h->dpt_fold = !(getenv("SKIMI_DPT_FOLD") && atoi(getenv("SKIMI_DPT_FOLD")) == 0);
+    h->keep_copy = getenv("SKIMI_KEEP_COPY") && atoi(getenv("SKIMI_KEEP_COPY")) != 0;
+    h->qkv_fused = !(getenv("SKIMI_QKV_FUSED") && atoi(getenv("SKIMI_QKV_FUSED")) == 0);
     return h;
 }
 
diff --git a/skiing_analysis_pytorch_amd/ops.py b/skiing_analysis_pytorch_amd/ops.py
--- a/skiing_analysis_pytorch_amd/ops.py
+++ b/skiing_analysis_pytorch_amd/ops.py
@@ -28,7 +28,9 @@
 def gemm(a, w, *, prec=PREC_BF16X3, bias=None, gamma=None, resid=None, act=ACT_NONE, out=None,
          out_dtype=torch.float32, conv=None, resid_map=None, pixel_shuffle=None, splitk_scratch=None,
          force_splitk=0, M=None, lda=None, w_split=None, x3_scratch=None, a_records=None, out_records=None,
-         records_only=False, post_act=ACT_NONE, resid2=None, out2=None, out_map=None, splitk_zeroed=False):
+         records_only=False, post_act=ACT_NONE, resid2=None, out2=None, out_map=None, splitk_zeroed=False,
+         qk_heads=0, qn_w=None, qn_b=None, kn_w=None, kn_b=None, qk_pos=None, rope_cos=None, rope_sin=None, qk_eps=1e-5,
+         q_scale=1.0):
     _require_cuda(w, bias, gamma, resid, out, resid2, out2)
     if out_map is not None and out is None:
         raise _lib.SkimiError("gemm: out_map needs a caller-owned out (the remapped rows cannot be sized here)")
@@ -107,6 +109,13 @@
     if out_records is not None:
         _require_cuda(out_records)
         d.out_records = ptr(out_records)
+    if qk_heads:
+        _require_cuda(qn_w, qn_b, kn_w, kn_b, qk_pos, rope_cos, rope_sin)
+        d.qk_epilogue, d.qk_heads = 1, qk_heads
+        d.qn_w, d.qn_b, d.kn_w, d.kn_b = ptr(qn_w), ptr(qn_b), ptr(kn_w), ptr(kn_b)
+        d.qk_pos, d.rope_cos, d.rope_sin = ptr(qk_pos), ptr(rope_cos), ptr(rope_sin)
+        d.rope_npos = rope_cos.shape[0] if rope_cos is not None else 0
+        d.qk_eps, d.q_scale = qk_eps, q_scale
     check(lib().skimi_gemm(C.byref(d), _lib.current_stream()), "skimi_gemm")
     return out
 
```

Result: no change. 18.11 (median of 6 runs) (+0.5%).
